# Shashank8834/multimodal-fl-security

Measured on AMD Instinct MI355X. Metric: FL rounds/sec + aggregate-ms, K=128 clients 10M-param multimodal, 1/2/4/8 GPU, higher is better.
Workload: dtype f32 (bf16x6-split MFMA conv/GEMM = fp32 operands; Krum Gram bf16x4 hi/lo split, fp32 accumulate); 1 GPU; C3: Multi-Krum K=128, 20% sign-flip, ResNet-18 img + 1-layer GRU text late fusion, 5 local SGD steps/round; Krum distances reference-exact; preset=C3, model=resnet18-img+gru1-text late-fusion, clients=128, params=11800394, local_steps=5, batch=32, defense=krum(f=25, multi_k=64), attack=sign_flip, attackers=25, client_chunk=128, exchange=alltoall, krum_distances=reference-exact (fp32 torch.norm accumulation, D bit-identical to krum.py:89-97), training_phase=one captured HIP graph per round; local updates = one flr_train_clients_ex call

## Files before the change

### multimodal-fl-security_amd/csrc/agg_pairwise_ref.hip

```cpp
#include <cstdint>
#include <type_traits>
#include <utility>
#include <vector>

#include "flr_common.h"

namespace flr {
namespace pwref {

typedef float f32x4 __attribute__((ext_vector_type(4)));
typedef int i32x16 __attribute__((ext_vector_type(16)));

constexpr int IW = 4;
constexpr int JW = 16;
constexpr int SB = 32;
constexpr int OFF_W = (SB / IW) * (SB / JW);
constexpr int DIAG_W = SB / IW;
constexpr int CS = 64;
constexpr int NQ = CS / 4;
constexpr int RPD = 256 / CS;
constexpr int SROWS = 20;
#ifndef FLR_REF_NSTAGE
#define FLR_REF_NSTAGE 8
#endif
constexpr int NSTAGE = FLR_REF_NSTAGE;
constexpr int STAGE = SROWS * CS;
constexpr int64_t XC_CAP = int64_t(8) << 30;
constexpr int64_t XC_SLACK = 4096;
constexpr int64_t XC_GROUP = (int64_t)NSTAGE * CS;
static_assert(CS == 64 && NQ == 16, "x_i layout: 16 lanes x 4 steps per chunk");
static_assert(NSTAGE % 2 == 0 && NSTAGE >= 4, "two register buffers");
static_assert((NSTAGE - 1) * CS * 4 <= XC_SLACK, "the prefetch past a stream stays inside the slack");
static_assert((NSTAGE - 1) * STAGE * 4 < 65536, "ds_read_b128's 16-bit offset reaches every stage");
static_assert(NSTAGE * STAGE * 4 > 163840 / 5, "LDS caps the CU at four workgroups: one wave per SIMD");
template <bool DIAG>
struct Staging {
  static constexpr int DPW = (DIAG ? SROWS : JW) / RPD;
  static constexpr int OPB = DPW + 1;
  static_assert((NSTAGE - 2) * OPB + 1 < 64, "vmcnt counts to 63");
};

__host__ __device__ constexpr int slot_swz(int row) { return row & 15; }

__host__ __device__ inline int tiles_before(int Y) { return DIAG_W * Y * Y; }
__host__ __device__ inline int ntiles_of(int K) { return tiles_before((K + SB - 1) / SB); }
struct Tile {
  int X, Y, g, h;
  bool diag;
};
__host__ __device__ inline Tile tile_of(int t) {
  int Y = 0;
  while (tiles_before(Y + 1) <= t) ++Y;
  const int local = t - tiles_before(Y);
  Tile r;
  r.Y = Y;
  if (local < Y * OFF_W) {
    r.X = local / OFF_W;
    r.g = (local % OFF_W) >> 1;
    r.h = local & 1;
    r.diag = false;
  } else {
    r.X = Y;
    r.g = local - Y * OFF_W;
    r.h = 0;
    r.diag = true;
  }
  return r;
}
__host__ __device__ inline int tile_of_pair(int i, int j) {
  const int X = i / SB, Y = j / SB;
  if (X < Y) return tiles_before(Y) + X * OFF_W + 2 * ((i % SB) / IW) + (j % SB) / JW;
  const int a = i % SB, b = j % SB, o = b - a;
  const int ii = o <= SB / 2 ? a : b;
  return tiles_before(Y) + Y * OFF_W + ii / IW;
}

constexpr int TW = 256;
constexpr int TROW = TW + 4;
struct WaveRuns {
  static constexpr int MAX = 48;
  int n;
  int64_t w0[MAX], pre[MAX + 1];
};
__global__ __launch_bounds__(256) void chain_transpose_kernel(const float* __restrict__ X, int64_t ldx, int64_t r0,
                                                              int64_t steps, int64_t ldc, float* __restrict__ Xc,
                                                              const WaveRuns runs) {
  __shared__ __attribute__((aligned(16))) float t[4 * 8 * TROW];
  const int k = blockIdx.y, wave = threadIdx.x >> 6, lane = threadIdx.x & 63;
  const int64_t q = (int64_t)blockIdx.x * 4 + wave;
  if (q >= runs.pre[runs.n]) return;
  int r = 0;
  while (q >= runs.pre[r + 1]) ++r;
  const int64_t s0 = (runs.w0[r] + q - runs.pre[r]) * TW;
  const int nv = (int)(steps - s0 < TW ? steps - s0 : TW);
  const float* src = X + (int64_t)k * ldx + 8 * (r0 + s0);
  float* tw = t + wave * 8 * TROW;
  const int h = lane & 1, sl = lane >> 1;
  f32x4 v[8];
  if (nv == TW) {
#pragma unroll
    for (int q = 0; q < 8; ++q) v[q] = __builtin_nontemporal_load(reinterpret_cast<const f32x4*>(src) + 64 * q + lane);
  } else {
#pragma unroll
    for (int q = 0; q < 8; ++q)
      v[q] = 32 * q + sl < nv ? reinterpret_cast<const f32x4*>(src)[64 * q + lane] : f32x4{0.f, 0.f, 0.f, 0.f};
  }
#pragma unroll
  for (int q = 0; q < 8; ++q)
#pragma unroll
    for (int e = 0; e < 4; ++e) tw[(4 * h + e) * TROW + 32 * q + sl] = v[q][e];
  asm volatile("s_waitcnt lgkmcnt(0)" ::: "memory");
  float* dst = Xc + (int64_t)k * 8 * ldc + s0 + 4 * lane;
  if (nv == TW) {
#pragma unroll
    for (int c = 0; c < 8; ++c)
      *reinterpret_cast<f32x4*>(dst + (int64_t)c * ldc) = *reinterpret_cast<const f32x4*>(tw + c * TROW + 4 * lane);
  } else {
    for (int c = 0; c < 8; ++c)
      for (int e = 0; e < 4 && 4 * lane + e < nv; ++e) dst[(int64_t)c * ldc + e] = tw[c * TROW + 4 * lane + e];
  }
}

constexpr int TAP_CO = 32;
constexpr int TAP_ROWS = 288;
static_assert(TAP_CO * TAP_ROWS < (1 << 14), "dense write items exact in fp32");
template <int KKT, bool VEC>
__global__ __launch_bounds__(256) void tap_chain_kernel(const float* __restrict__ X, int64_t ldx, int64_t off,
                                                        int Cout, int Cin, int KKr, int64_t r0, int64_t steps,
                                                        int64_t ldc, float* __restrict__ Xc,
                                                        const float* __restrict__ gdead, uint64_t dead, int nneg) {
  constexpr int TCO = TAP_CO, TROWS = TAP_ROWS;
  __shared__ float tile[TROWS][TCO + 1];
  const int KK = KKT > 0 ? KKT : KKr;
  const int CI = TROWS / KK;
  const int nci_t = (Cin + CI - 1) / CI, ntiles = (int)gridDim.x;
  const int x = (int)(blockIdx.x & 7), j = (int)(blockIdx.x >> 3);
  const int tl = x * (ntiles / 8) + min(x, ntiles % 8) + j;
  const int co0 = (tl / nci_t) * TCO, ci0 = (tl % nci_t) * CI;
  const int nci = min(CI, Cin - ci0), nco_v = min(TCO, Cout - co0);
  const int k = blockIdx.y;
  const float* row = X + (int64_t)k * ldx + off;
  const float* grow = gdead ? gdead + off : row;
  const float gs = k < nneg ? -1.f : 1.f;
  auto is_dead = [&](int t) { return t < 64 && ((dead >> t) & 1); };
  auto src = [&](int t) { return is_dead(t) ? grow : row; };
  auto sgn = [&](int t) { return is_dead(t) ? gs : 1.f; };
  const int nrows = KK * CI;
  if constexpr (VEC) {
    constexpr int LPR = TCO / 4, RPP = 256 / LPR;
    const int sub = threadIdx.x % LPR, rr = threadIdx.x / LPR;
    constexpr int IT = (TROWS + RPP - 1) / RPP;
    f32x4 v[IT];
#pragma unroll
    for (int q = 0; q < IT; ++q) {
      const int r = rr + RPP * q, t = r / CI, ci = r - t * CI;
      const int64_t e = ((int64_t)t * Cin + ci0 + ci) * Cout + co0 + 4 * sub;
      if (!(r < nrows && ci < nci))
        v[q] = f32x4{0.f, 0.f, 0.f, 0.f};
      else if (is_dead(t))
        v[q] = *reinterpret_cast<const f32x4*>(grow + e) * gs;
      else
        v[q] = __builtin_nontemporal_load(reinterpret_cast<const f32x4*>(row + e));
    }
#pragma unroll
    for (int q = 0; q < IT; ++q) {
      const int r = rr + RPP * q;
      if (r < nrows)
#pragma unroll
        for (int e = 0; e < 4; ++e) tile[r][4 * sub + e] = v[q][e];
    }
  } else {
    for (int e = threadIdx.x; e < nrows * TCO; e += 256) {
      const int co = e % TCO, r = e / TCO, t = r / CI, ci = r % CI;
      if (ci < nci && co < nco_v) tile[r][co] = src(t)[((int64_t)t * Cin + ci0 + ci) * Cout + co0 + co] * sgn(t);
    }
  }
  __syncthreads();
  const int64_t L = (int64_t)nci * KK;
  const int64_t ulo = 8 * r0, uhi = 8 * (r0 + steps);
  float* out = Xc + (int64_t)k * 8 * ldc;
  {
    const int64_t CL = (int64_t)Cin * KK;
    const int64_t ufirst = off + ((int64_t)co0 * Cin + ci0) * KK;
    if (CL % 8 == 0 && L % 8 == 0 && ufirst >= ulo && ufirst + (nco_v - 1) * CL + L <= uhi) {
      const int Li = (int)L, m = Li / 8, a0 = (int)(ufirst & 7);
      const int64_t sb0 = (ufirst >> 3) - r0, CLs = CL / 8;
      const float inv_L = 1.f / (float)Li, inv_m = 1.f / (float)m;
      const int n = nco_v * Li;
#pragma unroll 4
      for (int i = threadIdx.x; i < n; i += 256) {
        const int co = (int)(((float)i + 0.5f) * inv_L);
        const int q = i - co * Li;
        const int c = (int)(((float)q + 0.5f) * inv_m);
        const int jj = q - c * m;
        const int dc = (c - a0) & 7;
        const int rel = dc + 8 * jj, ci = rel / KK, t = rel - ci * KK;
        out[(int64_t)c * ldc + sb0 + co * CLs + ((a0 + dc) >> 3) + jj] = tile[t * CI + ci][co];
      }
      return;
    }
  }
  static_assert(TROWS / 8 + 1 <= 64, "a run's steps fit its slots");
#pragma unroll 4
  for (int i = threadIdx.x; i < nco_v * 512; i += 256) {
    const int ns = i & 63, c = (i >> 6) & 7, co = i >> 9;
    const int64_t u0 = off + ((int64_t)(co0 + co) * Cin + ci0) * KK;
    const int64_t u = 8 * ((u0 >> 3) + ns) + c;
    if (u >= u0 && u < u0 + L && u >= ulo && u < uhi) {
      const int rel = (int)(u - u0), ci = rel / KK, t = rel - ci * KK;
      out[(int64_t)c * ldc + ((u >> 3) - r0)] = tile[t * CI + ci][co];
    }
  }
}

#ifndef FLR_REF_ABL
#define FLR_REF_ABL 0
#endif
#if FLR_REF_ABL == 1
#define FLR_CHAIN16(A, B, C, D, NOP) \
  NOP \
  "v_sub_f32 %[t0], %[x0], %[j0]\n\t" \
  "v_sub_f32 %[t1], %[x1], %[j1]\n\t" \
  "v_fmac_f32 %[acc], %[t0], %[t0]\n\t" \
  "v_sub_f32 %[t2], %[x2], %[j2]\n\t" \
  "v_fmac_f32 %[acc], %[t1], %[t1]\n\t" \
  "v_sub_f32 %[t0], %[x3], %[j3]\n\t" \
  "v_fmac_f32 %[acc], %[t2], %[t2]\n\t" \
  "v_sub_f32 %[t1], %[x0], %[j4]\n\t" \
  "v_fmac_f32 %[acc], %[t0], %[t0]\n\t" \
  "v_sub_f32 %[t2], %[x1], %[j5]\n\t" \
  "v_fmac_f32 %[acc], %[t1], %[t1]\n\t" \
  "v_sub_f32 %[t0], %[x2], %[j6]\n\t" \
  "v_fmac_f32 %[acc], %[t2], %[t2]\n\t" \
  "v_sub_f32 %[t1], %[x3], %[j7]\n\t" \
  "v_fmac_f32 %[acc], %[t0], %[t0]\n\t" \
  "v_sub_f32 %[t2], %[x0], %[j8]\n\t" \
  "v_fmac_f32 %[acc], %[t1], %[t1]\n\t" \
  "v_sub_f32 %[t0], %[x1], %[j9]\n\t" \
  "v_fmac_f32 %[acc], %[t2], %[t2]\n\t" \
  "v_sub_f32 %[t1], %[x2], %[j10]\n\t" \
  "v_fmac_f32 %[acc], %[t0], %[t0]\n\t" \
  "v_sub_f32 %[t2], %[x3], %[j11]\n\t" \
  "v_fmac_f32 %[acc], %[t1], %[t1]\n\t" \
  "v_sub_f32 %[t0], %[x0], %[j12]\n\t" \
  "v_fmac_f32 %[acc], %[t2], %[t2]\n\t" \
  "v_sub_f32 %[t1], %[x1], %[j13]\n\t" \
  "v_fmac_f32 %[acc], %[t0], %[t0]\n\t" \
  "v_sub_f32 %[t2], %[x2], %[j14]\n\t" \
  "v_fmac_f32 %[acc], %[t1], %[t1]\n\t" \
  "v_sub_f32 %[t0], %[x3], %[j15]\n\t" \
  "v_fmac_f32 %[acc], %[t2], %[t2]\n\t" \
  "v_fmac_f32 %[acc], %[t0], %[t0]\n\t"
#else
#define FLR_CHAIN16(A, B, C, D, NOP) \
  NOP \
  "v_sub_f32_dpp %[t0], %[x0], %[j0] row_newbcast:" #A " row_mask:0xf bank_mask:0xf\n\t" \
  "v_sub_f32_dpp %[t1], %[x1], %[j1] row_newbcast:" #A " row_mask:0xf bank_mask:0xf\n\t" \
  "v_fmac_f32 %[acc], %[t0], %[t0]\n\t" \
  "v_sub_f32_dpp %[t2], %[x2], %[j2] row_newbcast:" #A " row_mask:0xf bank_mask:0xf\n\t" \
  "v_fmac_f32 %[acc], %[t1], %[t1]\n\t" \
  "v_sub_f32_dpp %[t0], %[x3], %[j3] row_newbcast:" #A " row_mask:0xf bank_mask:0xf\n\t" \
  "v_fmac_f32 %[acc], %[t2], %[t2]\n\t" \
  "v_sub_f32_dpp %[t1], %[x0], %[j4] row_newbcast:" #B " row_mask:0xf bank_mask:0xf\n\t" \
  "v_fmac_f32 %[acc], %[t0], %[t0]\n\t" \
  "v_sub_f32_dpp %[t2], %[x1], %[j5] row_newbcast:" #B " row_mask:0xf bank_mask:0xf\n\t" \
  "v_fmac_f32 %[acc], %[t1], %[t1]\n\t" \
  "v_sub_f32_dpp %[t0], %[x2], %[j6] row_newbcast:" #B " row_mask:0xf bank_mask:0xf\n\t" \
  "v_fmac_f32 %[acc], %[t2], %[t2]\n\t" \
  "v_sub_f32_dpp %[t1], %[x3], %[j7] row_newbcast:" #B " row_mask:0xf bank_mask:0xf\n\t" \
  "v_fmac_f32 %[acc], %[t0], %[t0]\n\t" \
  "v_sub_f32_dpp %[t2], %[x0], %[j8] row_newbcast:" #C " row_mask:0xf bank_mask:0xf\n\t" \
  "v_fmac_f32 %[acc], %[t1], %[t1]\n\t" \
  "v_sub_f32_dpp %[t0], %[x1], %[j9] row_newbcast:" #C " row_mask:0xf bank_mask:0xf\n\t" \
  "v_fmac_f32 %[acc], %[t2], %[t2]\n\t" \
  "v_sub_f32_dpp %[t1], %[x2], %[j10] row_newbcast:" #C " row_mask:0xf bank_mask:0xf\n\t" \
  "v_fmac_f32 %[acc], %[t0], %[t0]\n\t" \
  "v_sub_f32_dpp %[t2], %[x3], %[j11] row_newbcast:" #C " row_mask:0xf bank_mask:0xf\n\t" \
  "v_fmac_f32 %[acc], %[t1], %[t1]\n\t" \
  "v_sub_f32_dpp %[t0], %[x0], %[j12] row_newbcast:" #D " row_mask:0xf bank_mask:0xf\n\t" \
  "v_fmac_f32 %[acc], %[t2], %[t2]\n\t" \
  "v_sub_f32_dpp %[t1], %[x1], %[j13] row_newbcast:" #D " row_mask:0xf bank_mask:0xf\n\t" \
  "v_fmac_f32 %[acc], %[t0], %[t0]\n\t" \
  "v_sub_f32_dpp %[t2], %[x2], %[j14] row_newbcast:" #D " row_mask:0xf bank_mask:0xf\n\t" \
  "v_fmac_f32 %[acc], %[t1], %[t1]\n\t" \
  "v_sub_f32_dpp %[t0], %[x3], %[j15] row_newbcast:" #D " row_mask:0xf bank_mask:0xf\n\t" \
  "v_fmac_f32 %[acc], %[t2], %[t2]\n\t" \
  "v_fmac_f32 %[acc], %[t0], %[t0]\n\t"
#endif
#define FLR_CHAIN_BLOCK(b, A, B, C, D, NOP)                                                                 \
  asm volatile(FLR_CHAIN16(A, B, C, D, NOP)                                                                \
               : [acc] "+v"(acc), [t0] "=&v"(t0), [t1] "=&v"(t1), [t2] "=&v"(t2)                        \
               : [x0] "v"(xv[0]), [x1] "v"(xv[1]), [x2] "v"(xv[2]), [x3] "v"(xv[3]), [j0] "v"(v[4 * (b) + 0][0]), [j1] "v"(v[4 * (b) + 0][1]), [j2] "v"(v[4 * (b) + 0][2]), [j3] "v"(v[4 * (b) + 0][3]), [j4] "v"(v[4 * (b) + 1][0]), [j5] "v"(v[4 * (b) + 1][1]), [j6] "v"(v[4 * (b) + 1][2]), [j7] "v"(v[4 * (b) + 1][3]), [j8] "v"(v[4 * (b) + 2][0]), [j9] "v"(v[4 * (b) + 2][1]), [j10] "v"(v[4 * (b) + 2][2]), [j11] "v"(v[4 * (b) + 2][3]), [j12] "v"(v[4 * (b) + 3][0]), [j13] "v"(v[4 * (b) + 3][1]), [j14] "v"(v[4 * (b) + 3][2]), [j15] "v"(v[4 * (b) + 3][3]))
__device__ __forceinline__ float chain_chunk(f32x4 xv, const f32x4 (&v)[NQ], float acc) {
  static_assert(NQ == 16, "four blocks of 16 steps");
  float t0, t1, t2;
  FLR_CHAIN_BLOCK(0, 0, 1, 2, 3, "s_nop 1\n\t");
  FLR_CHAIN_BLOCK(1, 4, 5, 6, 7, "");
  FLR_CHAIN_BLOCK(2, 8, 9, 10, 11, "");
  FLR_CHAIN_BLOCK(3, 12, 13, 14, 15, "");
  return acc;
}
#undef FLR_CHAIN_BLOCK
#undef FLR_CHAIN16

#define FLR_STEP2(XA, XB, J, L, TA, TB, PA, PB) \
  "v_sub_f32_dpp %[" #TA "], %[" #XA "], %[" #J "] row_newbcast:" #L " row_mask:0xf bank_mask:0xf\n\t" \
  "v_sub_f32_dpp %[" #TB "], %[" #XB "], %[" #J "] row_newbcast:" #L " row_mask:0xf bank_mask:0xf\n\t" \
  "v_fmac_f32 %[acc], %[" #PA "], %[" #PA "]\n\t" \
  "v_fmac_f32 %[acc2], %[" #PB "], %[" #PB "]\n\t"
#define FLR_STEP2_FIRST(XA, XB, J, L, TA, TB) \
  "v_sub_f32_dpp %[" #TA "], %[" #XA "], %[" #J "] row_newbcast:" #L " row_mask:0xf bank_mask:0xf\n\t" \
  "v_sub_f32_dpp %[" #TB "], %[" #XB "], %[" #J "] row_newbcast:" #L " row_mask:0xf bank_mask:0xf\n\t"
#define FLR_CHAIN16_2(A, B, C, D, NOP) \
  NOP \
  FLR_STEP2_FIRST(x0, y0, j0, A, a0, b0) \
  FLR_STEP2(x1, y1, j1, A, a1, b1, a0, b0) FLR_STEP2(x2, y2, j2, A, a0, b0, a1, b1) \
  FLR_STEP2(x3, y3, j3, A, a1, b1, a0, b0) FLR_STEP2(x0, y0, j4, B, a0, b0, a1, b1) \
  FLR_STEP2(x1, y1, j5, B, a1, b1, a0, b0) FLR_STEP2(x2, y2, j6, B, a0, b0, a1, b1) \
  FLR_STEP2(x3, y3, j7, B, a1, b1, a0, b0) FLR_STEP2(x0, y0, j8, C, a0, b0, a1, b1) \
  FLR_STEP2(x1, y1, j9, C, a1, b1, a0, b0) FLR_STEP2(x2, y2, j10, C, a0, b0, a1, b1) \
  FLR_STEP2(x3, y3, j11, C, a1, b1, a0, b0) FLR_STEP2(x0, y0, j12, D, a0, b0, a1, b1) \
  FLR_STEP2(x1, y1, j13, D, a1, b1, a0, b0) FLR_STEP2(x2, y2, j14, D, a0, b0, a1, b1) \
  FLR_STEP2(x3, y3, j15, D, a1, b1, a0, b0) \
  "v_fmac_f32 %[acc], %[a1], %[a1]\n\t" \
  "v_fmac_f32 %[acc2], %[b1], %[b1]\n\t"
#define FLR_CHAIN_BLOCK2(b, A, B, C, D, NOP)                                                                   \
  asm volatile(FLR_CHAIN16_2(A, B, C, D, NOP)                                                                 \
               : [acc] "+v"(acc), [acc2] "+v"(acc2), [a0] "=&v"(a0), [b0] "=&v"(b0), [a1] "=&v"(a1),          \
                 [b1] "=&v"(b1)                                                                              \
               : [x0] "v"(xv[0]), [x1] "v"(xv[1]), [x2] "v"(xv[2]), [x3] "v"(xv[3]), [y0] "v"(yv[0]),           \
                 [y1] "v"(yv[1]), [y2] "v"(yv[2]), [y3] "v"(yv[3]), [j0] "v"(v[4 * (b) + 0][0]),              \
                 [j1] "v"(v[4 * (b) + 0][1]), [j2] "v"(v[4 * (b) + 0][2]), [j3] "v"(v[4 * (b) + 0][3]),        \
                 [j4] "v"(v[4 * (b) + 1][0]), [j5] "v"(v[4 * (b) + 1][1]), [j6] "v"(v[4 * (b) + 1][2]),        \
                 [j7] "v"(v[4 * (b) + 1][3]), [j8] "v"(v[4 * (b) + 2][0]), [j9] "v"(v[4 * (b) + 2][1]),        \
                 [j10] "v"(v[4 * (b) + 2][2]), [j11] "v"(v[4 * (b) + 2][3]), [j12] "v"(v[4 * (b) + 3][0]),     \
                 [j13] "v"(v[4 * (b) + 3][1]), [j14] "v"(v[4 * (b) + 3][2]), [j15] "v"(v[4 * (b) + 3][3]))
__device__ __forceinline__ void chain_chunk2(f32x4 xv, f32x4 yv, const f32x4 (&v)[NQ], float& acc, float& acc2) {
  float a0, b0, a1, b1;
  FLR_CHAIN_BLOCK2(0, 0, 1, 2, 3, "s_nop 1\n\t");
  FLR_CHAIN_BLOCK2(1, 4, 5, 6, 7, "");
  FLR_CHAIN_BLOCK2(2, 8, 9, 10, 11, "");
  FLR_CHAIN_BLOCK2(3, 12, 13, 14, 15, "");
}
#undef FLR_CHAIN_BLOCK2
#undef FLR_CHAIN16_2
#undef FLR_STEP2_FIRST
#undef FLR_STEP2

template <class F, int... U>
__device__ __forceinline__ void static_for(F&& f, std::integer_sequence<int, U...>) {
  (f(std::integral_constant<int, U>{}), ...);
}

template <bool DIAG, int NST = NSTAGE, bool TWO = false>
__device__ __forceinline__ void ref_chain_tile(float* lds, const Tile T, const int c, const float* __restrict__ Xc,
                                               int64_t ldc, int K, int64_t steps, int first,
                                               float* __restrict__ A) {
  using S = Staging<DIAG>;
  static_assert(!(TWO && DIAG), "two chains per lane on off-diagonal tiles only");
  static_assert(NST % 2 == 0 && NST >= 4, "two register buffers");
  constexpr int NXI = TWO ? 2 : 1;
  constexpr int OPB = S::DPW + NXI;
  static_assert((NST - 2) * OPB + NXI < 64, "vmcnt counts to 63");
  const int lane = threadIdx.x & 63, r = lane >> 4, jl = lane & 15;
  int i, j, srow;
  bool keep = true;
  if (DIAG) {
    const int a = IW * T.g + r, o = jl + 1;
    i = SB * T.X + a;
    j = SB * T.X + ((a + o) & (SB - 1));
    srow = r + jl;
    keep = o < SB / 2 || a < SB / 2;
  } else {
    i = SB * T.X + (TWO ? 2 * IW : IW) * T.g + r;
    j = SB * T.Y + JW * T.h + jl;
    srow = jl;
  }
  const int i2 = i + IW;
  const bool valid2 = TWO && i2 < K && j < K;
  const bool valid = keep && i < K && j < K;
  const int lo = i < j ? i : j, hi = i < j ? j : i;
  const int64_t rs = 8 * ldc;

  float acc = 0.f, acc2 = 0.f;
  if (!first) {
    const float* ap = A + ((int64_t)c * K + (lo < K ? lo : K - 1)) * K + (hi < K ? hi : K - 1);
    asm volatile("global_load_dword %0, %1, off\n\ts_waitcnt vmcnt(0)" : "=v"(acc) : "v"(ap) : "memory");
    acc = valid ? acc : 0.f;
    if constexpr (TWO) {
      const float* ap2 = A + ((int64_t)c * K + (i2 < K ? i2 : K - 1)) * K + (j < K ? j : K - 1);
      asm volatile("global_load_dword %0, %1, off\n\ts_waitcnt vmcnt(0)" : "=v"(acc2) : "v"(ap2) : "memory");
      acc2 = valid2 ? acc2 : 0.f;
    }
  }

  const int jrow0 = DIAG ? SB * T.X : min(SB * T.Y + JW * T.h, K - 1);
  const char* sbj = reinterpret_cast<const char*>(Xc + (int64_t)jrow0 * rs + (int64_t)c * ldc) - 2048;
  uint32_t voj[S::DPW];
#pragma unroll
  for (int u = 0; u < S::DPW; ++u) {
    const int s = RPD * u + lane / NQ;
    int gj = DIAG ? SB * T.X + ((IW * T.g + 1 + s) & (SB - 1)) : SB * T.Y + JW * T.h + s;
    gj = gj < K ? gj : K - 1;
    voj[u] = (uint32_t)((int64_t)(gj - jrow0) * rs * 4 + 16 * ((lane % NQ) ^ slot_swz(s)) - 1024 * (u - 2) + 2048);
  }
  const int irow0 = min(DIAG ? SB * T.X + IW * T.g : i - r, K - 1);
  const char* sbi = reinterpret_cast<const char*>(Xc + (int64_t)irow0 * rs + (int64_t)c * ldc);
  const uint32_t voi = (uint32_t)((int64_t)((i < K ? i : K - 1) - irow0) * rs * 4 + 16 * jl);
  const uint32_t voi2 = (uint32_t)((int64_t)((i2 < K ? i2 : K - 1) - irow0) * rs * 4 + 16 * jl);
  static_assert(XC_GROUP % (NST * CS) == 0, "trips inside the zero fill");
  const int ngroup = (int)((steps + NST * CS - 1) / (NST * CS));
  auto issue = [&](int ch, int slot, f32x4& x, f32x4& x2) {
    const int64_t co = (int64_t)ch * CS * 4;
    if (FLR_REF_ABL == 3) return;
    const char* sb = sbj + co;
    const uint32_t m = (uint32_t)(uintptr_t)lds + 4 * slot * STAGE + 2048;
#define FLR_DMA(n, off) "global_load_lds_dwordx4 %[v" #n "], %[sb] offset:" #off "\n\t"
    if constexpr (S::DPW == 5)
      asm volatile("s_mov_b32 m0, %[m]\n\ts_nop 0\n\t" FLR_DMA(0, -2048) FLR_DMA(1, -1024) FLR_DMA(2, 0)
                       FLR_DMA(3, 1024) FLR_DMA(4, 2048)
                   :
                   : [m] "s"(m), [sb] "s"(sb), [v0] "v"(voj[0]), [v1] "v"(voj[1]), [v2] "v"(voj[2]), [v3] "v"(voj[3]),
                     [v4] "v"(voj[S::DPW - 1])
                   : "memory");
    else
      asm volatile("s_mov_b32 m0, %[m]\n\ts_nop 0\n\t" FLR_DMA(0, -2048) FLR_DMA(1, -1024) FLR_DMA(2, 0)
                       FLR_DMA(3, 1024)
                   :
                   : [m] "s"(m), [sb] "s"(sb), [v0] "v"(voj[0]), [v1] "v"(voj[1]), [v2] "v"(voj[2]), [v3] "v"(voj[3])
                   : "memory");
#undef FLR_DMA
    static_assert(S::DPW == 4 || S::DPW == 5, "the DMA statements above");
    asm volatile("global_load_dwordx4 %0, %1, %2" : "=v"(x) : "v"(voi), "s"(sbi + co) : "memory");
    if constexpr (TWO) asm volatile("global_load_dwordx4 %0, %1, %2" : "=v"(x2) : "v"(voi2), "s"(sbi + co) : "memory");
  };
  const int rsw = slot_swz(srow);
  uint32_t ra[NQ];
#pragma unroll
  for (int q = 0; q < NQ; ++q) ra[q] = (uint32_t)(uintptr_t)(lds + srow * CS + 4 * (q ^ rsw));
  auto rows = [](auto st, f32x4(&v)[NQ], const uint32_t(&a)[NQ]) {
#pragma unroll
    for (int q = 0; q < NQ; ++q)
      if (FLR_REF_ABL != 2)
        asm volatile("ds_read_b128 %0, %1 offset:%2" : "=v"(v[q]) : "v"(a[q]), "n"(decltype(st)::value * STAGE * 4)
                     : "memory");
  };

  f32x4 va[NQ], vb[NQ];
  f32x4 xs[NST], xs2[NST];
  auto body = [&](auto U, int ch, f32x4(&vc)[NQ], f32x4(&vn)[NQ]) {
    constexpr int u = decltype(U)::value;
    asm volatile("s_waitcnt vmcnt(%0)" ::"n"((NST - 3) * OPB + NXI) : "memory");
    asm volatile("s_waitcnt lgkmcnt(0)" ::: "memory");
    asm volatile("" : "+v"(vc[0]), "+v"(vc[1]), "+v"(vc[2]), "+v"(vc[3]), "+v"(vc[4]), "+v"(vc[5]), "+v"(vc[6]),
                 "+v"(vc[7]), "+v"(vc[8]), "+v"(vc[9]), "+v"(vc[10]), "+v"(vc[11]), "+v"(vc[12]), "+v"(vc[13]),
                 "+v"(vc[14]), "+v"(vc[15]), "+v"(xs[u]));
    if constexpr (TWO) asm volatile("" : "+v"(xs2[u]));
    issue(ch + NST - 1, (u + NST - 1) % NST, xs[(u + NST - 1) % NST], xs2[(u + NST - 1) % NST]);
    rows(std::integral_constant<int, (u + 1) % NST>{}, vn, ra);
    if constexpr (TWO)
      chain_chunk2(xs[u], xs2[u], vc, acc, acc2);
    else if (FLR_REF_ABL != 5)
      acc = chain_chunk(xs[u], vc, acc);
  };
#pragma unroll
  for (int u = 0; u < NST - 1; ++u) issue(u, u, xs[u], xs2[u]);
  asm volatile("s_waitcnt vmcnt(%0)" ::"n"((NST - 2) * OPB + NXI) : "memory");
  rows(std::integral_constant<int, 0>{}, va, ra);
  for (int ch = 0; ch < ngroup * NST; ch += NST)
    static_for(
        [&](auto U) {
          constexpr int u = decltype(U)::value;
          if constexpr (u % 2 == 0)
            body(U, ch + u, va, vb);
          else
            body(U, ch + u, vb, va);
        },
        std::make_integer_sequence<int, NST>{});
  asm volatile("s_waitcnt vmcnt(0) lgkmcnt(0)" ::: "memory");
  if (valid) A[((int64_t)c * K + lo) * K + hi] = acc;
  if (valid2) A[((int64_t)c * K + i2) * K + j] = acc2;
}

__global__ __launch_bounds__(64) void ref_chain_kernel(const float* __restrict__ Xc, int64_t ldc, int K,
                                                       int64_t steps, int t0, int first, float* __restrict__ A) {
  __shared__ __attribute__((aligned(16))) float lds[NSTAGE * STAGE];
  const int c = (int)(blockIdx.x & 7);
  const Tile T = tile_of(t0 + (int)(blockIdx.x >> 3));
  if (T.diag)
    ref_chain_tile<true>(lds, T, c, Xc, ldc, K, steps, first, A);
  else
    ref_chain_tile<false>(lds, T, c, Xc, ldc, K, steps, first, A);
}

constexpr int NST2 = 4;
__host__ __device__ inline int tiles2_before(int Y) { return 4 * Y * (Y + 1); }
__host__ __device__ inline int ntiles2_of(int K) { return tiles2_before((K + SB - 1) / SB); }
__host__ __device__ inline Tile tile2_of(int t) {
  int Y = 0;
  while (tiles2_before(Y + 1) <= t) ++Y;
  const int local = t - tiles2_before(Y);
  Tile r;
  r.Y = Y;
  if (local < 8 * Y) {
    r.X = local / 8;
    r.g = (local % 8) >> 1;
    r.h = local & 1;
    r.diag = false;
  } else {
    r.X = Y;
    r.g = local - 8 * Y;
    r.h = 0;
    r.diag = true;
  }
  return r;
}
__global__ __launch_bounds__(64, 2) void ref_chain2_kernel(const float* __restrict__ Xc, int64_t ldc, int K,
                                                           int64_t steps, int first, float* __restrict__ A) {
  __shared__ __attribute__((aligned(16))) float lds[NST2 * STAGE];
  const int c = (int)(blockIdx.x & 7);
  const Tile T = tile2_of((int)(blockIdx.x >> 3));
  if (T.diag)
    ref_chain_tile<true, NST2, false>(lds, T, c, Xc, ldc, K, steps, first, A);
  else
    ref_chain_tile<false, NST2, true>(lds, T, c, Xc, ldc, K, steps, first, A);
}

inline bool use_two_chains(int64_t K) {
  const char* e = flr::knob("FLR_REF_2I");
  return e && e[0] == '1' && K > SB;
}

constexpr int QJ = 64;
constexpr int QTB = 16;
constexpr int QD = 8;
static_assert(XC_GROUP % (4 * QTB) == 0 && XC_GROUP % (4 * QD) == 0, "padded segments hold whole tiles / trips");
__host__ __device__ inline int64_t quad_rows(int64_t K) { return (K + QJ - 1) / QJ * QJ; }
__host__ __device__ inline int quad_ni(int q, int K, int ni) {
  const int a = QJ / ni * (q + 1), b = (K + ni - 1) / ni;
  return a < b ? a : b;
}
inline int64_t quad_slack(int64_t K) { return (QD + 4) * quad_rows(K) * 16; }
inline int quad_ntiles(int K, int ni) {
  int n = 0;
  for (int q = 0; q * QJ < K; ++q) n += quad_ni(q, K, ni);
  return n;
}

__global__ __launch_bounds__(256) void quad_transpose_kernel(const float* __restrict__ X, int64_t ldx, int K,
                                                             int64_t r0, int64_t steps, int64_t NB, int64_t Kp,
                                                             float* __restrict__ Xq) {
  __shared__ f32x4 t[QTB][QTB * 8 + 1];
  const int tid = threadIdx.x;
  const int64_t b0 = (int64_t)blockIdx.x * QTB;
  const int k0 = blockIdx.y * QTB;
  const int64_t u0 = 8 * (r0 + 4 * b0), uend = 8 * (r0 + steps);
  f32x4 v[8];
#pragma unroll
  for (int q = 0; q < 8; ++q) {
    const int idx = q * 256 + tid, row = idx >> 7, p = idx & 127;
    const int64_t u = u0 + 4 * p;
    v[q] = (k0 + row < K && u < uend)
               ? __builtin_nontemporal_load(reinterpret_cast<const f32x4*>(X + (int64_t)(k0 + row) * ldx + u))
               : f32x4{0.f, 0.f, 0.f, 0.f};
  }
#pragma unroll
  for (int q = 0; q < 8; ++q) {
    const int idx = q * 256 + tid;
    t[idx >> 7][idx & 127] = v[q];
  }
  __syncthreads();
  const int k = tid & 15, bl = tid >> 4;
  if (k0 + k >= K) return;
  f32x4 w[8];
#pragma unroll
  for (int q = 0; q < 8; ++q) w[q] = t[k][8 * bl + q];
  float* out = Xq + ((b0 + bl) * Kp + k0 + k) * 4;
#pragma unroll
  for (int c = 0; c < 8; ++c) {
    const int h = c >> 2, m = c & 3;
    *reinterpret_cast<f32x4*>(out + (int64_t)c * NB * Kp * 4) = f32x4{w[h][m], w[2 + h][m], w[4 + h][m], w[6 + h][m]};
  }
}

template <int E>
__device__ __forceinline__ void sgpr_step(float (&acc)[4], const i32x16& g0, const i32x16&, float xjv) {
  float t0, t1;
  asm volatile(
      "v_sub_f32 %[t0], %[s0], %[x]\n\t"
      "v_sub_f32 %[t1], %[s1], %[x]\n\t"
      "v_fmac_f32 %[a0], %[t0], %[t0]\n\t"
      "v_sub_f32 %[t0], %[s2], %[x]\n\t"
      "v_fmac_f32 %[a1], %[t1], %[t1]\n\t"
      "v_sub_f32 %[t1], %[s3], %[x]\n\t"
      "v_fmac_f32 %[a2], %[t0], %[t0]\n\t"
      "v_fmac_f32 %[a3], %[t1], %[t1]\n\t"
      : [a0] "+v"(acc[0]), [a1] "+v"(acc[1]), [a2] "+v"(acc[2]), [a3] "+v"(acc[3]), [t0] "=&v"(t0), [t1] "=&v"(t1)
      : [s0] "s"(g0[E]), [s1] "s"(g0[4 + E]), [s2] "s"(g0[8 + E]), [s3] "s"(g0[12 + E]), [x] "v"(xjv));
}
template <int E>
__device__ __forceinline__ void sgpr_step(float (&acc)[8], const i32x16& g0, const i32x16& g1, float xjv) {
  float t0, t1;
  asm volatile(
      "v_sub_f32 %[t0], %[s0], %[x]\n\t"
      "v_sub_f32 %[t1], %[s1], %[x]\n\t"
      "v_fmac_f32 %[a0], %[t0], %[t0]\n\t"
      "v_sub_f32 %[t0], %[s2], %[x]\n\t"
      "v_fmac_f32 %[a1], %[t1], %[t1]\n\t"
      "v_sub_f32 %[t1], %[s3], %[x]\n\t"
      "v_fmac_f32 %[a2], %[t0], %[t0]\n\t"
      "v_sub_f32 %[t0], %[s4], %[x]\n\t"
      "v_fmac_f32 %[a3], %[t1], %[t1]\n\t"
      "v_sub_f32 %[t1], %[s5], %[x]\n\t"
      "v_fmac_f32 %[a4], %[t0], %[t0]\n\t"
      "v_sub_f32 %[t0], %[s6], %[x]\n\t"
      "v_fmac_f32 %[a5], %[t1], %[t1]\n\t"
      "v_sub_f32 %[t1], %[s7], %[x]\n\t"
      "v_fmac_f32 %[a6], %[t0], %[t0]\n\t"
      "v_fmac_f32 %[a7], %[t1], %[t1]\n\t"
      : [a0] "+v"(acc[0]), [a1] "+v"(acc[1]), [a2] "+v"(acc[2]), [a3] "+v"(acc[3]), [a4] "+v"(acc[4]),
        [a5] "+v"(acc[5]), [a6] "+v"(acc[6]), [a7] "+v"(acc[7]), [t0] "=&v"(t0), [t1] "=&v"(t1)
      : [s0] "s"(g0[E]), [s1] "s"(g0[4 + E]), [s2] "s"(g0[8 + E]), [s3] "s"(g0[12 + E]), [s4] "s"(g1[E]),
        [s5] "s"(g1[4 + E]), [s6] "s"(g1[8 + E]), [s7] "s"(g1[12 + E]), [x] "v"(xjv));
}

#ifndef FLR_REF_S_ABL
#define FLR_REF_S_ABL 0
#endif
template <int NI, int BT>
__global__ __launch_bounds__(64) void ref_chain_s_kernel(const float* __restrict__ Xq, int64_t NB, int64_t Kp, int K,
                                                         int first, float* __restrict__ A) {
  static_assert(NI == 4 || NI == 8, "the step forms above");
  constexpr int NL = NI * BT / 4;
  static_assert(QD % (2 * BT) == 0, "whole ping-pong pairs of buffers per trip");
  const int c = (int)(blockIdx.x & 7), lane = threadIdx.x;
  int t = (int)(blockIdx.x >> 3), q = 0;
  for (int n = quad_ni(0, K, NI); t >= n; n = quad_ni(q, K, NI)) {
    t -= n;
    ++q;
  }
  const int i0 = NI * t, j = QJ * q + lane;
  const float* __restrict__ base = Xq + (int64_t)c * NB * Kp * 4;
  float acc[NI];
  if (first) {
#pragma unroll
    for (int r = 0; r < NI; ++r) acc[r] = 0.f;
  } else {
#pragma unroll
    for (int r = 0; r < NI; ++r) {
      const float* ap = A + ((int64_t)c * K + i0 + r) * K + (j < K ? j : K - 1);
      asm volatile("global_load_dword %0, %1, off" : "=v"(acc[r]) : "v"(ap) : "memory");
    }
    if constexpr (NI == 4)
      asm volatile("s_waitcnt vmcnt(0)" : "+v"(acc[0]), "+v"(acc[1]), "+v"(acc[2]), "+v"(acc[3]) : : "memory");
    else
      asm volatile("s_waitcnt vmcnt(0)"
                   : "+v"(acc[0]), "+v"(acc[1]), "+v"(acc[2]), "+v"(acc[3]), "+v"(acc[4]), "+v"(acc[5]),
                     "+v"(acc[6]), "+v"(acc[7])
                   :
                   : "memory");
#pragma unroll
    for (int r = 0; r < NI; ++r) acc[r] = (i0 + r < j && j < K) ? acc[r] : 0.f;
  }
  const int64_t bb = Kp * 16;
  const uint32_t voff = (uint32_t)j * 16;
  const char* pjn = reinterpret_cast<const char*>(base);
  const char* pin = reinterpret_cast<const char*>(base) + (int64_t)i0 * 16;
  auto ldj = [&](f32x4& x) {
    asm volatile("global_load_dwordx4 %0, %1, %2" : "=v"(x) : "v"(voff), "s"(pjn) : "memory");
    pjn += bb;
    asm volatile("" : "+s"(pjn));
  };
  auto ldi = [&](i32x16(&buf)[NL]) {
    const char* pu = pin;
#pragma unroll
    for (int u = 0; u < BT; ++u) {
#pragma unroll
      for (int h = 0; h < NI / 4; ++h)
        asm volatile("s_load_dwordx16 %0, %1, %2" : "=s"(buf[u * (NI / 4) + h]) : "s"(pu), "n"(64 * h) : "memory");
      pu += bb;
      asm volatile("" : "+s"(pu));
    }
    pin = pu;
  };
  f32x4 xj[QD];
  i32x16 xa[NL], xb[NL];
#pragma unroll
  for (int u = 0; u < QD; ++u) ldj(xj[u]);
  ldi(xa);
  auto trip = [&](auto U0, const i32x16(&cur)[NL], i32x16(&nxt)[NL]) {
    constexpr int u0 = decltype(U0)::value;
    if (FLR_REF_S_ABL != 2 && FLR_REF_S_ABL != 4) asm volatile("s_waitcnt lgkmcnt(0)" ::: "memory");
    if (FLR_REF_S_ABL != 2) ldi(nxt);
#pragma unroll
    for (int v = 0; v < BT; ++v) {
      f32x4& x = xj[u0 + v];
      if (FLR_REF_S_ABL != 1) asm volatile("s_waitcnt vmcnt(%0)" ::"n"(QD - 1) : "memory");
      asm volatile("" : "+v"(x));
      const i32x16& g0 = cur[v * (NI / 4)];
      const i32x16& g1 = cur[v * (NI / 4) + (NI / 4) - 1];
      if (FLR_REF_S_ABL != 3) {
        sgpr_step<0>(acc, g0, g1, x[0]);
        sgpr_step<1>(acc, g0, g1, x[1]);
        sgpr_step<2>(acc, g0, g1, x[2]);
        sgpr_step<3>(acc, g0, g1, x[3]);
      }
      if (FLR_REF_S_ABL != 1) ldj(x);
    }
  };
  for (int64_t b0 = 0; b0 < NB; b0 += QD)
    static_for(
        [&](auto P) {
          constexpr int p = decltype(P)::value;
          trip(std::integral_constant<int, 2 * BT * p>{}, xa, xb);
          trip(std::integral_constant<int, 2 * BT * p + BT>{}, xb, xa);
        },
        std::make_integer_sequence<int, QD / (2 * BT)>{});
  asm volatile("s_waitcnt vmcnt(0) lgkmcnt(0)" ::: "memory");
#pragma unroll
  for (int r = 0; r < NI; ++r) {
    const int i = i0 + r;
    if (i < j && j < K) A[((int64_t)c * K + i) * K + j] = acc[r];
  }
}

constexpr int WCB = 8;
constexpr int WNS = 4;
static_assert(WCB % 8 == 0 && (XC_GROUP / 4) % WCB == 0, "two DMAs per wave per chunk; whole chunks per segment");
__host__ __device__ inline int wg_groups(int q, int K) { return (quad_ni(q, K, 8) + 3) / 4; }
inline int wg_ntiles(int K) {
  int n = 0;
  for (int q = 0; q * QJ < K; ++q) n += wg_groups(q, K);
  return n;
}
template <int E>
__device__ __forceinline__ void vgpr_step(float (&acc)[8], const f32x4 (&xi)[8], float xjv) {
  float t0, t1;
  asm volatile(
      "v_sub_f32 %[t0], %[s0], %[x]\n\t"
      "v_sub_f32 %[t1], %[s1], %[x]\n\t"
      "v_fmac_f32 %[a0], %[t0], %[t0]\n\t"
      "v_sub_f32 %[t0], %[s2], %[x]\n\t"
      "v_fmac_f32 %[a1], %[t1], %[t1]\n\t"
      "v_sub_f32 %[t1], %[s3], %[x]\n\t"
      "v_fmac_f32 %[a2], %[t0], %[t0]\n\t"
      "v_sub_f32 %[t0], %[s4], %[x]\n\t"
      "v_fmac_f32 %[a3], %[t1], %[t1]\n\t"
      "v_sub_f32 %[t1], %[s5], %[x]\n\t"
      "v_fmac_f32 %[a4], %[t0], %[t0]\n\t"
      "v_sub_f32 %[t0], %[s6], %[x]\n\t"
      "v_fmac_f32 %[a5], %[t1], %[t1]\n\t"
      "v_sub_f32 %[t1], %[s7], %[x]\n\t"
      "v_fmac_f32 %[a6], %[t0], %[t0]\n\t"
      "v_fmac_f32 %[a7], %[t1], %[t1]\n\t"
      : [a0] "+v"(acc[0]), [a1] "+v"(acc[1]), [a2] "+v"(acc[2]), [a3] "+v"(acc[3]), [a4] "+v"(acc[4]),
        [a5] "+v"(acc[5]), [a6] "+v"(acc[6]), [a7] "+v"(acc[7]), [t0] "=&v"(t0), [t1] "=&v"(t1)
      : [s0] "v"(xi[0][E]), [s1] "v"(xi[1][E]), [s2] "v"(xi[2][E]), [s3] "v"(xi[3][E]), [s4] "v"(xi[4][E]),
        [s5] "v"(xi[5][E]), [s6] "v"(xi[6][E]), [s7] "v"(xi[7][E]), [x] "v"(xjv));
}

template <bool XL>
__global__ __launch_bounds__(256, 3) void ref_chain_w_kernel(const float* __restrict__ Xq, int64_t NB, int64_t Kp,
                                                             int K, int first, float* __restrict__ A) {
  constexpr int SJ = WCB * QJ * 16;
  constexpr int SI = XL ? WCB * 32 * 16 : 0;
  constexpr int NDMA = XL ? 3 : 2;
  __shared__ __attribute__((aligned(16))) float xs[WNS * (SJ + SI) / 4];
  const int c = (int)(blockIdx.x & 7), lane = threadIdx.x & 63;
  const int wave = __builtin_amdgcn_readfirstlane((int)(threadIdx.x >> 6));
  int t = (int)(blockIdx.x >> 3), q = 0;
  for (int n = wg_groups(0, K); t >= n; n = wg_groups(q, K)) {
    t -= n;
    ++q;
  }
  const int a = 4 * t + wave, na = quad_ni(q, K, 8);
  const bool live = a < na;
  const int i0 = 8 * (live ? a : na - 1), j = QJ * q + lane;
  const float* __restrict__ base = Xq + (int64_t)c * NB * Kp * 4;
  float acc[8];
  if (first || !live) {
#pragma unroll
    for (int r = 0; r < 8; ++r) acc[r] = 0.f;
  } else {
#pragma unroll
    for (int r = 0; r < 8; ++r) {
      const float* ap = A + ((int64_t)c * K + i0 + r) * K + (j < K ? j : K - 1);
      asm volatile("global_load_dword %0, %1, off" : "=v"(acc[r]) : "v"(ap) : "memory");
    }
    asm volatile("s_waitcnt vmcnt(0)"
                 : "+v"(acc[0]), "+v"(acc[1]), "+v"(acc[2]), "+v"(acc[3]), "+v"(acc[4]), "+v"(acc[5]), "+v"(acc[6]),
                   "+v"(acc[7])
                 :
                 : "memory");
#pragma unroll
    for (int r = 0; r < 8; ++r) acc[r] = (i0 + r < j && j < K) ? acc[r] : 0.f;
  }
  const int64_t bb = Kp * 16;
  const int64_t nch = NB / WCB;
  const char* jsrc = reinterpret_cast<const char*>(base) + (int64_t)(QJ * q) * 16;
  const char* isrc = reinterpret_cast<const char*>(base) + (int64_t)(32 * t) * 16;
  const uint32_t vj = (uint32_t)lane * 16;
  const uint32_t vi = (uint32_t)(((lane >> 5) * Kp + (lane & 31)) * 16);
  const uint32_t lds0 = (uint32_t)(uintptr_t)xs;
  auto dma = [&](int64_t ch) {
    const int64_t cc = ch < nch ? ch : nch - 1;
    const uint32_t sb = lds0 + (uint32_t)((int)(ch % WNS) * (SJ + SI));
#pragma unroll
    for (int v = 0; v < 2; ++v) {
      const int blk = 2 * wave + v;
      const char* src = jsrc + (cc * WCB + blk) * bb;
      const uint32_t m = sb + (uint32_t)(blk * QJ * 16);
      asm volatile("s_mov_b32 m0, %[m]\n\ts_nop 0\n\tglobal_load_lds_dwordx4 %[v], %[s] offset:0"
                   :
                   : [m] "s"(m), [v] "v"(vj), [s] "s"(src)
                   : "memory");
    }
    if constexpr (XL) {
      const char* src = isrc + (cc * WCB + 2 * wave) * bb;
      const uint32_t m = sb + SJ + (uint32_t)(2 * wave * 32 * 16);
      asm volatile("s_mov_b32 m0, %[m]\n\ts_nop 0\n\tglobal_load_lds_dwordx4 %[v], %[s] offset:0"
                   :
                   : [m] "s"(m), [v] "v"(vi), [s] "s"(src)
                   : "memory");
    }
  };
  const char* pin = reinterpret_cast<const char*>(base) + (int64_t)i0 * 16;
  auto ldi = [&](i32x16& lo, i32x16& hi) {
    asm volatile("s_load_dwordx16 %0, %2, 0x0\n\ts_load_dwordx16 %1, %2, 0x40" : "=s"(lo), "=s"(hi) : "s"(pin) : "memory");
    pin += bb;
    asm volatile("" : "+s"(pin));
  };
  auto rdj = [&](f32x4& x, uint32_t addr, auto U) {
    asm volatile("ds_read_b128 %0, %1 offset:%2" : "=v"(x) : "v"(addr), "n"(decltype(U)::value * QJ * 16) : "memory");
  };
  auto rdi = [&](f32x4(&x)[8], uint32_t addr, auto U) {
#pragma unroll
    for (int r = 0; r < 8; ++r)
      asm volatile("ds_read_b128 %0, %1 offset:%2"
                   : "=v"(x[r])
                   : "v"(addr), "n"(SJ + decltype(U)::value * 32 * 16 + 16 * r)
                   : "memory");
  };
  i32x16 al, ah, bl, bh;
  f32x4 j0, j1, ia[8], ib[8];
#pragma unroll
  for (int p = 0; p < WNS - 1; ++p) dma(p);
  if constexpr (!XL) ldi(al, ah);
  auto body = [&](auto U, uint32_t sbase, uint32_t ibase, f32x4& xc, f32x4& xn, const i32x16& cl,
                  const i32x16& ch_, i32x16& nl, i32x16& nh, f32x4(&ic)[8], f32x4(&in)[8]) {
    constexpr int u = decltype(U)::value;
    if constexpr (XL) {
      asm volatile("s_waitcnt lgkmcnt(0)"
                   : "+v"(xc), "+v"(ic[0]), "+v"(ic[1]), "+v"(ic[2]), "+v"(ic[3]), "+v"(ic[4]), "+v"(ic[5]),
                     "+v"(ic[6]), "+v"(ic[7])
                   :
                   : "memory");
      if constexpr (u + 1 < WCB) {
        rdj(xn, sbase, std::integral_constant<int, u + 1>{});
        rdi(in, ibase, std::integral_constant<int, u + 1>{});
      }
      vgpr_step<0>(acc, ic, xc[0]);
      vgpr_step<1>(acc, ic, xc[1]);
      vgpr_step<2>(acc, ic, xc[2]);
      vgpr_step<3>(acc, ic, xc[3]);
    } else {
      asm volatile("s_waitcnt lgkmcnt(0)" : "+v"(xc) : : "memory");
      ldi(nl, nh);
      if constexpr (u + 1 < WCB) rdj(xn, sbase, std::integral_constant<int, u + 1>{});
      sgpr_step<0>(acc, cl, ch_, xc[0]);
      sgpr_step<1>(acc, cl, ch_, xc[1]);
      sgpr_step<2>(acc, cl, ch_, xc[2]);
      sgpr_step<3>(acc, cl, ch_, xc[3]);
    }
  };
  static_assert(WCB % 2 == 0, "x_i / x_j ping-pong");
  for (int64_t ch = 0; ch < nch; ++ch) {
    asm volatile("s_waitcnt vmcnt(%0)\n\ts_barrier" ::"n"(NDMA * (WNS - 2)) : "memory");
    dma(ch + WNS - 1);
    const uint32_t st = lds0 + (uint32_t)((int)(ch % WNS) * (SJ + SI));
    const uint32_t sbase = st + vj;
    const uint32_t ibase = st + (uint32_t)(wave * 8 * 16);
    rdj(j0, sbase, std::integral_constant<int, 0>{});
    if constexpr (XL) rdi(ia, ibase, std::integral_constant<int, 0>{});
    static_for(
        [&](auto P) {
          constexpr int p = decltype(P)::value;
          body(std::integral_constant<int, 2 * p>{}, sbase, ibase, j0, j1, al, ah, bl, bh, ia, ib);
          body(std::integral_constant<int, 2 * p + 1>{}, sbase, ibase, j1, j0, bl, bh, al, ah, ib, ia);
        },
        std::make_integer_sequence<int, WCB / 2>{});
  }
  asm volatile("s_waitcnt vmcnt(0) lgkmcnt(0)" ::: "memory");
  if (live) {
#pragma unroll
    for (int r = 0; r < 8; ++r) {
      const int i = i0 + r;
      if (i < j && j < K) A[((int64_t)c * K + i) * K + j] = acc[r];
    }
  }
}

inline bool use_quad(int64_t K, int64_t ntaps, bool all_tiles) {
  if (!all_tiles || ntaps > 0 || K <= QJ) return false;
  const char* e = flr::knob("FLR_REF_SGPR");
  if (e && e[0] == '0') return false;
  if (e && e[0] == '1') return true;
  return K >= 480;
}

struct TailCols {
  int64_t c[8];
};
__global__ void ref_finish_kernel(const float* __restrict__ A, int chains, const float* __restrict__ X,
                                  const TailCols tc, int K, int64_t P, int64_t ldx, int64_t R, int t0, int t1,
                                  double* __restrict__ D) {
  const int64_t idx = (int64_t)blockIdx.x * blockDim.x + threadIdx.x;
  if (idx >= (int64_t)K * K) return;
  const int i = (int)(idx / K), j = (int)(idx % K);
  if (i == j) {
    D[idx] = 0.0;
    return;
  }
  if (i > j) return;
  const int tile = tile_of_pair(i, j);
  double v = 0.0;
  if (tile >= t0 && tile < t1) {
    float s = 0.f;
    if (chains) {
      const int64_t kk = (int64_t)K * K, p = (int64_t)i * K + j;
      s = A[p];
#pragma unroll
      for (int c = 1; c < 8; ++c) s = add_rn(s, A[c * kk + p]);
    }
    const float* xi = X + (int64_t)i * ldx;
    const float* xj = X + (int64_t)j * ldx;
    int64_t t = R * 8;
    auto col = [&](int64_t c) { return tc.c[c - R * 8]; };
    if (t + 4 <= P)
      for (const int64_t e = t + 4; t < e; ++t) {
        const float d = xi[col(t)] - xj[col(t)];
        s = add_rn(s, mul_rn(d, d));
      }
    for (; t < P; ++t) {
      const float d = xi[col(t)] - xj[col(t)];
      s = __builtin_fmaf(d, d, s);
    }
    v = (double)sqrt_rn(s);
  }
  D[(int64_t)i * K + j] = v;
  D[(int64_t)j * K + i] = v;
}

inline size_t a_bytes(int64_t K) { return align_up((size_t)(8 * K * K) * 4, 256); }

}
}

using namespace flr;
using namespace flr::pwref;

extern "C" size_t flr_pairwise_l2_reference_workspace(int64_t K, int64_t P) {
  if (K < 1 || P < 0) return 0;
  const int64_t R = P / 8;
  size_t n = a_bytes(K);
  if (K < 2 || R == 0) return n;
  const int64_t Rc = (R + XC_GROUP - 1) / XC_GROUP * XC_GROUP;
  const int64_t per_step = (K > QJ ? quad_rows(K) : K) * 8 * 4;
  const int64_t nseg = (per_step * Rc + XC_CAP - 1) / XC_CAP;
  const int64_t Rs = ((R + nseg - 1) / nseg + XC_GROUP - 1) / XC_GROUP * XC_GROUP;
  return n + (size_t)(per_step * Rs + XC_SLACK + (K > QJ ? quad_slack(K) : 0));
}

extern "C" int flr_pairwise_l2_reference_tiles(int64_t K) {
  if (K < 2 || K > (1 << 15)) return 0;
  return ntiles_of((int)K);
}

static WaveRuns wave_runs(const int64_t* taps, int64_t ntaps, int64_t r0, int64_t steps) {
  const int64_t nw = (steps + TW - 1) / TW;
  std::vector<std::pair<int64_t, int64_t>> v;
  int64_t b = 0;
  for (int64_t w = 0; w < nw; ++w) {
    const int64_t u0 = 8 * (r0 + w * TW), u1 = u0 + 8 * TW;
    while (b < ntaps && taps[4 * b] + taps[4 * b + 1] * taps[4 * b + 2] * taps[4 * b + 3] <= u0) ++b;
    const bool inside = b < ntaps && u0 >= taps[4 * b] &&
                        u1 <= taps[4 * b] + taps[4 * b + 1] * taps[4 * b + 2] * taps[4 * b + 3];
    if (inside) continue;
    if (!v.empty() && v.back().second == w)
      v.back().second = w + 1;
    else
      v.push_back({w, w + 1});
  }
  while ((int)v.size() > WaveRuns::MAX) {
    size_t best = 1;
    for (size_t i = 2; i < v.size(); ++i)
      if (v[i].first - v[i - 1].second < v[best].first - v[best - 1].second) best = i;
    v[best - 1].second = v[best].second;
    v.erase(v.begin() + (int64_t)best);
  }
  WaveRuns wr;
  wr.n = (int)v.size();
  wr.pre[0] = 0;
  for (int i = 0; i < wr.n; ++i) {
    wr.w0[i] = v[i].first;
    wr.pre[i + 1] = wr.pre[i] + (v[i].second - v[i].first);
  }
  return wr;
}

static int run_chains(const float* X, int64_t K, int64_t steps_total, int64_t ldx, const int64_t* taps, int64_t ntaps,
                      const uint64_t* dead, const float* gdead, int64_t nneg, int first, float* A, void* ws,
                      size_t ws_bytes, int t0, int t1, hipStream_t st) {
  const size_t na = a_bytes(K);
  if (ws_bytes < na) return FLR_ERR_WORKSPACE;
  const int64_t R = steps_total;
  if (ws_bytes < na + (size_t)XC_SLACK) return FLR_ERR_WORKSPACE;
  if (use_quad(K, ntaps, t0 == 0 && t1 == ntiles_of((int)K))) {
    const int64_t Kp = quad_rows(K), qstep = Kp * 8 * 4;
    const char* rows_knob = flr::knob("FLR_REF_SGPR_ROWS");
    const bool eight = rows_knob && rows_knob[0] == '8';
    const char* form_knob = flr::knob("FLR_REF_SGPR_FORM");
    const bool wg = !(form_knob && form_knob[0] == 'w' && form_knob[1] == 'a');
    const bool xl = !(form_knob && form_knob[0] == 's');
    if (ws_bytes < na + (size_t)(XC_SLACK + quad_slack(K))) return FLR_ERR_WORKSPACE;
    const int64_t cap =
        (int64_t)((ws_bytes - na - XC_SLACK - quad_slack(K)) / (size_t)qstep) / XC_GROUP * XC_GROUP;
    if (cap < XC_GROUP) return FLR_ERR_WORKSPACE;
    const int64_t nseg = (R + cap - 1) / cap;
    const int64_t Rs = ((R + nseg - 1) / nseg + XC_GROUP - 1) / XC_GROUP * XC_GROUP;
    float* Xq = reinterpret_cast<float*>(reinterpret_cast<char*>(ws) + na);
    for (int64_t seg = 0; seg < nseg; ++seg) {
      const int64_t r0 = seg * Rs, steps = (R - r0 < Rs) ? R - r0 : Rs;
      if (steps <= 0) break;
      const int64_t NB = (steps + XC_GROUP - 1) / XC_GROUP * XC_GROUP / 4;
      hipLaunchKernelGGL(quad_transpose_kernel, dim3((unsigned)(NB / QTB), (unsigned)((K + QTB - 1) / QTB)), dim3(256),
                         0, st, X, ldx, (int)K, r0, steps, NB, Kp, Xq);
      int rc = launch_status("quad_transpose_kernel");
      if (rc != FLR_OK) return rc;
      const int fst = (first && seg == 0) ? 1 : 0;
      if (wg && xl)
        hipLaunchKernelGGL(ref_chain_w_kernel<true>, dim3((unsigned)(8 * wg_ntiles((int)K))), dim3(256), 0, st, Xq, NB,
                           Kp, (int)K, fst, A);
      else if (wg)
        hipLaunchKernelGGL(ref_chain_w_kernel<false>, dim3((unsigned)(8 * wg_ntiles((int)K))), dim3(256), 0, st, Xq,
                           NB, Kp, (int)K, fst, A);
      else if (eight)
        hipLaunchKernelGGL((ref_chain_s_kernel<8, 1>), dim3((unsigned)(8 * quad_ntiles((int)K, 8))), dim3(64), 0, st,
                           Xq, NB, Kp, (int)K, fst, A);
      else
        hipLaunchKernelGGL((ref_chain_s_kernel<4, 2>), dim3((unsigned)(8 * quad_ntiles((int)K, 4))), dim3(64), 0, st,
                           Xq, NB, Kp, (int)K, fst, A);
      if ((rc = launch_status("ref_chain_s_kernel")) != FLR_OK) return rc;
    }
    return FLR_OK;
  }
  const int64_t per_step = K * 8 * 4;
  const int64_t ldc = (int64_t)((ws_bytes - na - XC_SLACK) / (size_t)per_step) / XC_GROUP * XC_GROUP;
  if (ldc < XC_GROUP) return FLR_ERR_WORKSPACE;
  const int64_t nseg = (R + ldc - 1) / ldc;
  const int64_t Rs = ((R + nseg - 1) / nseg + XC_GROUP - 1) / XC_GROUP * XC_GROUP;
  float* Xc = reinterpret_cast<float*>(reinterpret_cast<char*>(ws) + na);
  for (int64_t seg = 0; seg < nseg; ++seg) {
    const int64_t r0 = seg * Rs, steps = (R - r0 < Rs) ? R - r0 : Rs;
    if (steps <= 0) break;
    const WaveRuns runs = wave_runs(taps, ntaps, r0, steps);
    int rc = FLR_OK;
    if (runs.pre[runs.n] > 0) {
      hipLaunchKernelGGL(chain_transpose_kernel, dim3((unsigned)((runs.pre[runs.n] + 3) / 4), (unsigned)K), dim3(256),
                         0, st, X, ldx, r0, steps, ldc, Xc, runs);
      if ((rc = launch_status("chain_transpose_kernel")) != FLR_OK) return rc;
    }
    for (int64_t b = 0; b < ntaps; ++b) {
      const int64_t off = taps[4 * b], co = taps[4 * b + 1], ci = taps[4 * b + 2], kk = taps[4 * b + 3];
      if (off + co * ci * kk <= 8 * r0 || off >= 8 * (r0 + steps)) continue;
      const int64_t tiles = (co + TAP_CO - 1) / TAP_CO * ((ci + TAP_ROWS / kk - 1) / (TAP_ROWS / kk));
      const bool vec = off % 4 == 0 && co % TAP_CO == 0;
      auto kern = kk == 9 ? (vec ? tap_chain_kernel<9, true> : tap_chain_kernel<9, false>)
                : kk == 1 ? (vec ? tap_chain_kernel<1, true> : tap_chain_kernel<1, false>)
                          : (vec ? tap_chain_kernel<0, true> : tap_chain_kernel<0, false>);
      const uint64_t dm = dead ? dead[b] : 0;
      hipLaunchKernelGGL(kern, dim3((unsigned)tiles, (unsigned)K), dim3(256), 0, st, X, ldx, off, (int)co, (int)ci,
                         (int)kk, r0, steps, ldc, Xc, dm ? gdead : nullptr, dm, (int)std::min<int64_t>(nneg, K));
      if ((rc = launch_status("tap_chain_kernel")) != FLR_OK) return rc;
    }
    const int64_t padded = (steps + XC_GROUP - 1) / XC_GROUP * XC_GROUP;
    if (padded > steps &&
        hipMemset2DAsync(Xc + steps, (size_t)ldc * 4, 0, (size_t)(padded - steps) * 4, (size_t)(K * 8), st) != hipSuccess)
      return FLR_ERR_HIP;
    if (t0 == 0 && t1 == ntiles_of((int)K) && use_two_chains(K)) {
      hipLaunchKernelGGL(ref_chain2_kernel, dim3(8 * ntiles2_of((int)K)), dim3(64), 0, st, Xc, ldc, (int)K, steps,
                         (first && seg == 0) ? 1 : 0, A);
      rc = launch_status("ref_chain2_kernel");
    } else {
      hipLaunchKernelGGL(ref_chain_kernel, dim3(8 * (t1 - t0)), dim3(64), 0, st, Xc, ldc, (int)K, steps, t0,
                         (first && seg == 0) ? 1 : 0, A);
      rc = launch_status("ref_chain_kernel");
    }
    if (rc != FLR_OK) return rc;
  }
  return FLR_OK;
}

static int check_rows(const float* X, int64_t K, int64_t n, int64_t ldx) {
  if (K > 1 && n >= 8 && (((reinterpret_cast<uintptr_t>(X) & 15) != 0) || (ldx % 4) != 0)) return FLR_ERR_ARG;
  return FLR_OK;
}

extern "C" int flr_pairwise_l2_reference_tap_dead(const float* X, int64_t K, int64_t P, int64_t ldx,
                                                  const int64_t* taps, int64_t ntaps, const uint64_t* dead,
                                                  const float* gdead, int64_t nneg, double* D, void* ws,
                                                  size_t ws_bytes, int64_t part, int64_t nparts, void* stream) {
  if (K < 1 || P < 0 || ldx < P || !D || (K > 1 && P > 0 && !X) || nparts < 1 || part < 0 || part >= nparts)
    return FLR_ERR_ARG;
  if (K > (1 << 15)) return FLR_ERR_UNSUPPORTED;
  if (ntaps < 0 || (ntaps > 0 && !taps) || nneg < 0) return FLR_ERR_ARG;
  bool any_dead = false;
  for (int64_t b = 0; dead && b < ntaps; ++b) {
    if (taps[4 * b + 3] < 64 && (dead[b] >> taps[4 * b + 3]) != 0) return FLR_ERR_ARG;
    any_dead |= dead[b] != 0;
  }
  if (any_dead && !gdead) return FLR_ERR_ARG;
  for (int64_t b = 0, end = 0; b < ntaps; ++b) {
    const int64_t off = taps[4 * b], co = taps[4 * b + 1], ci = taps[4 * b + 2], kk = taps[4 * b + 3];
    if (off < end || co < 1 || ci < 1 || kk < 1 || kk > TAP_ROWS || co > INT32_MAX || ci > INT32_MAX ||
        off + co * ci * kk > P)
      return FLR_ERR_ARG;
    end = off + co * ci * kk;
  }
  int rc = check_rows(X, K, P, ldx);
  if (rc != FLR_OK) return rc;
  hipStream_t st = as_stream(stream);
  const int64_t R = P / 8;
  if (K > 1 && R > 0 && (!ws || (reinterpret_cast<uintptr_t>(ws) & 255) != 0)) return FLR_ERR_WORKSPACE;
  const int ntiles = K > 1 ? ntiles_of((int)K) : 0;
  const int t0 = (int)(part * ntiles / nparts), t1 = (int)((part + 1) * ntiles / nparts);
  float* A = reinterpret_cast<float*>(ws);
  if (K > 1 && R > 0 && t1 > t0 &&
      (rc = run_chains(X, K, R, ldx, taps, ntaps, any_dead ? dead : nullptr, gdead, nneg, 1, A, ws, ws_bytes, t0, t1,
                       st)) != FLR_OK)
    return rc;
  TailCols tc;
  for (int64_t u = 8 * R; u < 8 * R + 8; ++u) {
    int64_t c = u;
    for (int64_t b = 0; b < ntaps && u < P; ++b) {
      const int64_t off = taps[4 * b], co = taps[4 * b + 1], ci = taps[4 * b + 2], kk = taps[4 * b + 3];
      if (u < off || u >= off + co * ci * kk) continue;
      const int64_t rel = u - off, o = rel / (ci * kk), i = (rel / kk) % ci, t = rel % kk;
      c = off + (t * ci + i) * co + o;
    }
    tc.c[u - 8 * R] = c;
  }
  for (int64_t u = 8 * R; any_dead && u < P; ++u)
    for (int64_t b = 0; b < ntaps; ++b) {
      const int64_t off = taps[4 * b], co = taps[4 * b + 1], ci = taps[4 * b + 2], kk = taps[4 * b + 3];
      if (u < off || u >= off + co * ci * kk) continue;
      const int64_t t = (u - off) % kk;
      if (t < 64 && ((dead[b] >> t) & 1)) return FLR_ERR_ARG;
    }
  const int64_t kk = K * K;
  hipLaunchKernelGGL(ref_finish_kernel, dim3((unsigned)((kk + 255) / 256)), dim3(256), 0, st, A, R > 0 ? 1 : 0, X, tc,
                     (int)K, P, ldx, R, t0, t1, D);
  return launch_status("ref_finish_kernel");
}

extern "C" int flr_pairwise_l2_reference_tap(const float* X, int64_t K, int64_t P, int64_t ldx,
                                             const int64_t* taps, int64_t ntaps, double* D, void* ws, size_t ws_bytes,
                                             int64_t part, int64_t nparts, void* stream) {
  return flr_pairwise_l2_reference_tap_dead(X, K, P, ldx, taps, ntaps, nullptr, nullptr, 0, D, ws, ws_bytes, part,
                                            nparts, stream);
}

extern "C" int flr_pairwise_l2_reference(const float* X, int64_t K, int64_t P, int64_t ldx, double* D, void* ws,
                                         size_t ws_bytes, int64_t part, int64_t nparts, void* stream) {
  return flr_pairwise_l2_reference_tap(X, K, P, ldx, nullptr, 0, D, ws, ws_bytes, part, nparts, stream);
}

extern "C" int flr_pairwise_l2_reference_partial_tap(const float* X, int64_t K, int64_t steps, int64_t ldx,
                                                     const int64_t* taps, int64_t ntaps, int first, void* ws,
                                                     size_t ws_bytes, void* stream) {
  if (K < 1 || steps < 0 || ldx < 8 * steps || (K > 1 && steps > 0 && !X)) return FLR_ERR_ARG;
  if (ntaps < 0 || (ntaps > 0 && !taps)) return FLR_ERR_ARG;
  for (int64_t b = 0, end = 0; b < ntaps; ++b) {
    const int64_t off = taps[4 * b], co = taps[4 * b + 1], ci = taps[4 * b + 2], kk = taps[4 * b + 3];
    if (off < end || co < 1 || ci < 1 || kk < 1 || kk > TAP_ROWS || co > INT32_MAX || ci > INT32_MAX ||
        off + co * ci * kk > 8 * steps)
      return FLR_ERR_ARG;
    end = off + co * ci * kk;
  }
  if (K > (1 << 15)) return FLR_ERR_UNSUPPORTED;
  int rc = check_rows(X, K, 8 * steps, ldx);
  if (rc != FLR_OK) return rc;
  if (!ws || (reinterpret_cast<uintptr_t>(ws) & 255) != 0 || ws_bytes < a_bytes(K)) return FLR_ERR_WORKSPACE;
  hipStream_t st = as_stream(stream);
  float* A = reinterpret_cast<float*>(ws);
  if (K < 2) return FLR_OK;
  if (steps == 0) {
    if (first && hipMemsetAsync(A, 0, (size_t)8 * K * K * 4, st) != hipSuccess)
      return launch_status("reference distances: zero the chains");
    return FLR_OK;
  }
  return run_chains(X, K, steps, ldx, taps, ntaps, nullptr, nullptr, 0, first, A, ws, ws_bytes, 0, ntiles_of((int)K),
                    st);
}

extern "C" int flr_pairwise_l2_reference_partial(const float* X, int64_t K, int64_t steps, int64_t ldx, int first,
                                                 void* ws, size_t ws_bytes, void* stream) {
  return flr_pairwise_l2_reference_partial_tap(X, K, steps, ldx, nullptr, 0, first, ws, ws_bytes, stream);
}

extern "C" int flr_pairwise_l2_reference_finish(const float* Xtail, int64_t K, int64_t ntail, int64_t ldx,
                                                int chains, const void* ws, double* D, void* stream) {
  if (K < 1 || ntail < 0 || ntail > 7 || ldx < ntail || !D || (K > 1 && ntail > 0 && !Xtail) ||
      (K > 1 && chains && !ws))
    return FLR_ERR_ARG;
  if (K > (1 << 15)) return FLR_ERR_UNSUPPORTED;
  TailCols tc;
  for (int u = 0; u < 8; ++u) tc.c[u] = u;
  const int64_t kk = K * K;
  hipLaunchKernelGGL(ref_finish_kernel, dim3((unsigned)((kk + 255) / 256)), dim3(256), 0, as_stream(stream),
                     reinterpret_cast<const float*>(ws), chains ? 1 : 0, Xtail, tc, (int)K, ntail, ldx, (int64_t)0, 0,
                     K > 1 ? ntiles_of((int)K) : 0, D);
  return launch_status("ref_finish_kernel");
}
```

Measured before the change: 15.64 rounds/s.

## Compact dead-tap columns out of Krum chain and stream shared dead values separately

For conv taps whose per-client values come from a shared global (dead) tensor with a sign flip, the live taps are now packed separately in the transposed chain buffer. The dead taps are written once into a shared stream with the doubled value, rather than copied per client. A new dead-pattern chain kernel reads that stream into LDS by DMA and adds its squared terms only for mixed-sign client pairs, pointing other pairs at a zero block. The aim is to cut per-client transpose traffic and chain FMAs on dead taps while keeping the distance accumulation order exact. The cost is much more complexity: region planning, hand-scheduled asm specialised for two tap masks, and an Inf/NaN flag passed to the finish kernel.

```diff
diff --git a/multimodal-fl-security_amd/csrc/agg_pairwise_ref.hip b/multimodal-fl-security_amd/csrc/agg_pairwise_ref.hip
--- a/multimodal-fl-security_amd/csrc/agg_pairwise_ref.hip
+++ b/multimodal-fl-security_amd/csrc/agg_pairwise_ref.hip
@@ -124,15 +124,29 @@
 constexpr int TAP_CO = 32;
 constexpr int TAP_ROWS = 288;
 static_assert(TAP_CO * TAP_ROWS < (1 << 14), "dense write items exact in fp32");
-template <int KKT, bool VEC>
+
+struct DeadPlan {
+  int on;
+  int nl, nd;
+  uint64_t tap, rank;
+};
+__host__ __device__ inline int dead_nib(uint64_t v, int n) { return (int)((v >> (4 * n)) & 15); }
+__host__ __device__ inline int64_t dead_slot(int64_t rel, int t, int n, uint64_t rank) {
+  const int64_t c = rel & 7, s = rel >> 3;
+  return (s + 8 - c) / 9 * n + dead_nib(rank, t);
+}
+
+template <int KKT, bool VEC, bool CMP = false>
 __global__ __launch_bounds__(256) void tap_chain_kernel(const float* __restrict__ X, int64_t ldx, int64_t off,
                                                         int Cout, int Cin, int KKr, int64_t r0, int64_t steps,
                                                         int64_t ldc, float* __restrict__ Xc,
-                                                        const float* __restrict__ gdead, uint64_t dead, int nneg) {
+                                                        const float* __restrict__ gdead, uint64_t dead, int nneg,
+                                                        const DeadPlan dp) {
   constexpr int TCO = TAP_CO, TROWS = TAP_ROWS;
   __shared__ float tile[TROWS][TCO + 1];
   const int KK = KKT > 0 ? KKT : KKr;
-  const int CI = TROWS / KK;
+  const int NR = CMP ? dp.nl : KK;
+  const int CI = TROWS / NR;
   const int nci_t = (Cin + CI - 1) / CI, ntiles = (int)gridDim.x;
   const int x = (int)(blockIdx.x & 7), j = (int)(blockIdx.x >> 3);
   const int tl = x * (ntiles / 8) + min(x, ntiles % 8) + j;
@@ -145,7 +159,8 @@
   auto is_dead = [&](int t) { return t < 64 && ((dead >> t) & 1); };
   auto src = [&](int t) { return is_dead(t) ? grow : row; };
   auto sgn = [&](int t) { return is_dead(t) ? gs : 1.f; };
-  const int nrows = KK * CI;
+  const int nrows = NR * CI;
+  auto tap_of = [&](int tr) { return CMP ? dead_nib(dp.tap, tr) : tr; };
   if constexpr (VEC) {
     constexpr int LPR = TCO / 4, RPP = 256 / LPR;
     const int sub = threadIdx.x % LPR, rr = threadIdx.x / LPR;
@@ -153,11 +168,11 @@
     f32x4 v[IT];
 #pragma unroll
     for (int q = 0; q < IT; ++q) {
-      const int r = rr + RPP * q, t = r / CI, ci = r - t * CI;
+      const int r = rr + RPP * q, tr = r / CI, ci = r - tr * CI, t = tap_of(tr);
       const int64_t e = ((int64_t)t * Cin + ci0 + ci) * Cout + co0 + 4 * sub;
       if (!(r < nrows && ci < nci))
         v[q] = f32x4{0.f, 0.f, 0.f, 0.f};
-      else if (is_dead(t))
+      else if (!CMP && is_dead(t))
         v[q] = *reinterpret_cast<const f32x4*>(grow + e) * gs;
       else
         v[q] = __builtin_nontemporal_load(reinterpret_cast<const f32x4*>(row + e));
@@ -171,11 +186,24 @@
     }
   } else {
     for (int e = threadIdx.x; e < nrows * TCO; e += 256) {
-      const int co = e % TCO, r = e / TCO, t = r / CI, ci = r % CI;
-      if (ci < nci && co < nco_v) tile[r][co] = src(t)[((int64_t)t * Cin + ci0 + ci) * Cout + co0 + co] * sgn(t);
+      const int co = e % TCO, r = e / TCO, t = tap_of(r / CI), ci = r % CI;
+      if (ci < nci && co < nco_v)
+        tile[r][co] = (CMP ? row : src(t))[((int64_t)t * Cin + ci0 + ci) * Cout + co0 + co] * (CMP ? 1.f : sgn(t));
     }
   }
   __syncthreads();
+  if constexpr (CMP) {
+    const int per = nci * dp.nl, n = nco_v * per, p8 = per / 8;
+    const bool deal = per % 8 == 0;
+    float* outl = Xc + (int64_t)k * 8 * ldc;
+    for (int i = threadIdx.x; i < n; i += 256) {
+      const int co = i / per, l = i - co * per, q = deal ? 8 * (l % p8) + l / p8 : l;
+      const int ci = q / dp.nl, lt = q - ci * dp.nl, t = dead_nib(dp.tap, lt);
+      const int64_t rel = ((int64_t)(co0 + co) * Cin + ci0 + ci) * KK + t;
+      outl[(rel & 7) * ldc + dead_slot(rel, t, dp.nl, dp.rank)] = tile[lt * CI + ci][co];
+    }
+    return;
+  }
   const int64_t L = (int64_t)nci * KK;
   const int64_t ulo = 8 * r0, uhi = 8 * (r0 + steps);
   float* out = Xc + (int64_t)k * 8 * ldc;
@@ -352,15 +380,158 @@
   (f(std::integral_constant<int, U>{}), ...);
 }
 
-template <bool DIAG, int NST = NSTAGE, bool TWO = false>
+__global__ __launch_bounds__(256) void zero_slots_kernel(float* __restrict__ Xc, int64_t ldc, int n0, int64_t z0,
+                                                         int64_t z1) {
+  float* row = Xc + (int64_t)blockIdx.x * ldc;
+  const int n = n0 + (int)(z1 - z0);
+  for (int i = threadIdx.x; i < n; i += 256) row[i < n0 ? i : z0 + (i - n0)] = 0.f;
+}
+
+__global__ __launch_bounds__(256) void dead_stream_kernel(const float* __restrict__ g, int64_t off, int Cout, int Cin,
+                                                          const DeadPlan dp, int64_t ldt, float* __restrict__ T,
+                                                          int* __restrict__ flag) {
+  const int64_t idx = (int64_t)blockIdx.x * blockDim.x + threadIdx.x;
+  if (idx >= (int64_t)Cout * Cin * dp.nd) return;
+  const int64_t q = idx / dp.nd;
+  const int t = dead_nib(dp.tap, (int)(idx - q * dp.nd));
+  const int64_t co = q / Cin, ci = q - co * Cin;
+  const float v = g[off + ((int64_t)t * Cin + ci) * Cout + co];
+  if ((__float_as_uint(v) & 0x7f800000u) == 0x7f800000u) *flag = 1;
+  const int64_t rel = q * 9 + t;
+  T[(rel & 7) * ldt + dead_slot(rel, t, dp.nd, dp.rank)] = v + v;
+}
+
+template <int DM>
+struct DeadPat {
+  static constexpr int ND = __builtin_popcount(DM & 0x1ff), NL = 9 - ND;
+  static_assert(ND > 0 && NL > 0 && CS % NL == 0, "whole periods per chunk");
+  static constexpr int PPC = CS / NL;
+  static constexpr int TCH = PPC * ND;
+  static_assert(TCH % 4 == 0, "16-B reads of the dead stream");
+  static constexpr int NQT = TCH / 4;
+  static constexpr int NT = (TCH * 4 + 1023) / 1024;
+  static constexpr bool dead_at(int w) { return (DM >> (8 - w)) & 1; }
+  static constexpr int dead_before(int w) {
+    int n = 0;
+    for (int x = 0; x < w; ++x) n += dead_at(x) ? 1 : 0;
+    return n;
+  }
+};
+constexpr int NSTD = 4;
+#define FLR_FMA(x) "v_fmac_f32 %[acc], %[" #x "], %[" #x "]\n\t"
+#define FLR_SUB(dd, x, j, L) \
+  "v_sub_f32_dpp %[" #dd "], %[" #x "], %[" #j "] row_newbcast:%[" #L "] row_mask:0xf bank_mask:0xf\n\t"
+template <int DM>
+__device__ __forceinline__ float dead_chunk(f32x4 xv, const f32x4 (&v)[NQ], float acc, uint32_t ta) {
+  using Pt = DeadPat<DM>;
+  static_assert(DM == 0x1EF || DM == 0x04F, "the period statements below");
+  constexpr int ND = Pt::ND, NQT = Pt::NQT;
+  constexpr int RQ = NQT < 20 ? NQT : (DM == 0x1EF ? 14 : 20);
+  f32x4 tq[RQ];
+  float d[3];
+  auto readq = [&tq, &ta](auto Q) {
+    constexpr int q = decltype(Q)::value;
+    (void)tq, (void)ta;
+    asm volatile("ds_read_b128 %0, %1 offset:%2" : "=v"(tq[q % RQ]) : "v"(ta), "n"(16 * q) : "memory");
+  };
+  static_for([&readq](auto Q) { readq(Q); }, std::make_integer_sequence<int, RQ>{});
+  asm volatile("s_nop 1\n\t" FLR_SUB(da, x0, j0, L) FLR_SUB(db, x1, j1, L)
+               : [da] "=&v"(d[0]), [db] "=&v"(d[1])
+               : [x0] "v"(xv[0]), [x1] "v"(xv[1]), [j0] "v"(v[0][0]), [j1] "v"(v[0][1]), [L] "n"(0));
+  constexpr int G = DM == 0x1EF ? 2 : 1;
+  static_assert(Pt::PPC % G == 0, "whole groups per chunk");
+  static_for(
+      [&tq, &d, &acc, &readq, &xv, &v](auto PP) {
+        constexpr int pg = decltype(PP)::value, p = G * pg, n0 = ND * p;
+        (void)tq, (void)d, (void)acc, (void)xv, (void)v;
+        constexpr int done = n0 / 4, last = (done + RQ < NQT ? done + RQ : NQT) - 1, need = (n0 + G * ND - 1) / 4;
+        constexpr int cnt = last - need < 15 ? last - need : 15;
+        static_assert(need <= last, "the group's reads were issued");
+#define FLR_T(n) tq[((n0 + (n)) / 4) % RQ][(n0 + (n)) % 4]
+#define FLR_T8(a, b) [t##a##0] "v"(FLR_T(b + 0)), [t##a##1] "v"(FLR_T(b + 1)), [t##a##2] "v"(FLR_T(b + 2)), \
+                     [t##a##3] "v"(FLR_T(b + 3)), [t##a##4] "v"(FLR_T(b + 4)), [t##a##5] "v"(FLR_T(b + 5)), \
+                     [t##a##6] "v"(FLR_T(b + 6)), [t##a##7] "v"(FLR_T(b + 7))
+        if constexpr (DM == 0x1EF) {
+          constexpr int S = p, N = S + 2 < CS ? S + 2 : 0;
+          if constexpr (S + 2 < CS)
+            asm volatile("s_waitcnt lgkmcnt(%[w])\n\t" FLR_FMA(ta0) FLR_FMA(ta1) FLR_FMA(ta2) FLR_FMA(ta3) FLR_FMA(d0)
+                             FLR_SUB(n0, x0, j0, L0) FLR_FMA(ta4) FLR_FMA(ta5) FLR_FMA(ta6) FLR_FMA(ta7)
+                                 FLR_FMA(tb0) FLR_FMA(tb1) FLR_FMA(tb2) FLR_FMA(tb3) FLR_FMA(d1)
+                                     FLR_SUB(d0, x1, j1, L1) FLR_FMA(tb4) FLR_FMA(tb5) FLR_FMA(tb6) FLR_FMA(tb7)
+                         : [acc] "+v"(acc), [d0] "+v"(d[S % 3]), [d1] "+v"(d[(S + 1) % 3]), [n0] "=&v"(d[(S + 2) % 3])
+                         : [x0] "v"(xv[N % 4]), [j0] "v"(v[N / 4][N % 4]), [L0] "n"(N / 4), [x1] "v"(xv[(N + 1) % 4]),
+                           [j1] "v"(v[(N + 1) / 4][(N + 1) % 4]), [L1] "n"((N + 1) / 4), [w] "n"(cnt), FLR_T8(a, 0),
+                           FLR_T8(b, 8));
+          else
+            asm volatile("s_waitcnt lgkmcnt(%[w])\n\t" FLR_FMA(ta0) FLR_FMA(ta1) FLR_FMA(ta2) FLR_FMA(ta3) FLR_FMA(d0)
+                             FLR_FMA(ta4) FLR_FMA(ta5) FLR_FMA(ta6) FLR_FMA(ta7) FLR_FMA(tb0) FLR_FMA(tb1)
+                                 FLR_FMA(tb2) FLR_FMA(tb3) FLR_FMA(d1) FLR_FMA(tb4) FLR_FMA(tb5) FLR_FMA(tb6)
+                                     FLR_FMA(tb7)
+                         : [acc] "+v"(acc)
+                         : [d0] "v"(d[S % 3]), [d1] "v"(d[(S + 1) % 3]), [w] "n"(cnt), FLR_T8(a, 0), FLR_T8(b, 8));
+        } else {
+          constexpr int S = 4 * p;
+          float &da = d[S % 3], &db = d[(S + 1) % 3], &dc = d[(S + 2) % 3];
+          if constexpr (S + 4 < CS)
+            asm volatile("s_waitcnt lgkmcnt(%[w])\n\t" FLR_FMA(da) FLR_SUB(dc, x2, j2, L0) FLR_FMA(db)
+                             FLR_SUB(da, x3, j3, L0) FLR_FMA(t0) FLR_FMA(dc) FLR_SUB(db, x0, j4, L1) FLR_FMA(da)
+                                 FLR_SUB(dc, x1, j5, L1) FLR_FMA(t1) FLR_FMA(t2) FLR_FMA(t3) FLR_FMA(t4)
+                         : [acc] "+v"(acc), [da] "+v"(da), [db] "+v"(db), [dc] "+v"(dc)
+                         : [x0] "v"(xv[0]), [x1] "v"(xv[1]), [x2] "v"(xv[2]), [x3] "v"(xv[3]), [j2] "v"(v[p][2]),
+                           [j3] "v"(v[p][3]), [j4] "v"(v[p + 1 < NQ ? p + 1 : p][0]),
+                           [j5] "v"(v[p + 1 < NQ ? p + 1 : p][1]), [L0] "n"(p), [L1] "n"(p + 1), [w] "n"(cnt),
+                           [t0] "v"(FLR_T(0)), [t1] "v"(FLR_T(1)), [t2] "v"(FLR_T(2)), [t3] "v"(FLR_T(3)),
+                           [t4] "v"(FLR_T(4)));
+          else
+            asm volatile("s_waitcnt lgkmcnt(%[w])\n\t" FLR_FMA(da) FLR_SUB(dc, x2, j2, L0) FLR_FMA(db)
+                             FLR_SUB(da, x3, j3, L0) FLR_FMA(t0) FLR_FMA(dc) FLR_FMA(da) FLR_FMA(t1) FLR_FMA(t2)
+                                 FLR_FMA(t3) FLR_FMA(t4)
+                         : [acc] "+v"(acc), [da] "+v"(da), [db] "+v"(db), [dc] "+v"(dc)
+                         : [x2] "v"(xv[2]), [x3] "v"(xv[3]), [j2] "v"(v[p][2]), [j3] "v"(v[p][3]), [L0] "n"(p),
+                           [w] "n"(cnt), [t0] "v"(FLR_T(0)), [t1] "v"(FLR_T(1)), [t2] "v"(FLR_T(2)),
+                           [t3] "v"(FLR_T(3)), [t4] "v"(FLR_T(4)));
+        }
+#undef FLR_T8
+#undef FLR_T
+        static_for(
+            [&readq](auto E) {
+              constexpr int q = done + decltype(E)::value;
+              if constexpr (4 * q + 3 < n0 + G * ND && q + RQ < NQT) readq(std::integral_constant<int, q + RQ>{});
+            },
+            std::make_integer_sequence<int, (G * ND + 3) / 4 + 1>{});
+      },
+      std::make_integer_sequence<int, Pt::PPC / G>{});
+  return acc;
+}
+#undef FLR_SUB
+#undef FLR_FMA
+
+template <bool DIAG, int NST = NSTAGE, bool TWO = false, int DM = 0>
 __device__ __forceinline__ void ref_chain_tile(float* lds, const Tile T, const int c, const float* __restrict__ Xc,
-                                               int64_t ldc, int K, int64_t steps, int first,
-                                               float* __restrict__ A) {
+                                               int64_t ldc, int K, int64_t steps, int first, float* __restrict__ A,
+                                               const float* __restrict__ Tc = nullptr, int nneg = 0) {
   using S = Staging<DIAG>;
   static_assert(!(TWO && DIAG), "two chains per lane on off-diagonal tiles only");
   static_assert(NST % 2 == 0 && NST >= 4, "two register buffers");
+  constexpr int NT = [] {
+    if constexpr (DM != 0)
+      return DeadPat<DM>::NT;
+    else
+      return 0;
+  }();
+  constexpr int TCH = [] {
+    if constexpr (DM != 0)
+      return DeadPat<DM>::TCH;
+    else
+      return 0;
+  }();
+  static_assert(NT <= 2 && !(TWO && DM), "the dead stream's DMA statements below");
+  constexpr int STG = STAGE + NT * 256;
+  constexpr int ZERO = NST * STG;
+  static_assert((ZERO + NT * 256) * 4 <= NSTAGE * STAGE * 4, "inside the kernel's one LDS array");
+  static_assert((NST - 1) * STG * 4 < 65536, "ds_read_b128's 16-bit offset reaches every stage");
   constexpr int NXI = TWO ? 2 : 1;
-  constexpr int OPB = S::DPW + NXI;
+  constexpr int OPB = S::DPW + NT + NXI;
   static_assert((NST - 2) * OPB + NXI < 64, "vmcnt counts to 63");
   const int lane = threadIdx.x & 63, r = lane >> 4, jl = lane & 15;
   int i, j, srow;
@@ -404,6 +575,7 @@
     gj = gj < K ? gj : K - 1;
     voj[u] = (uint32_t)((int64_t)(gj - jrow0) * rs * 4 + 16 * ((lane % NQ) ^ slot_swz(s)) - 1024 * (u - 2) + 2048);
   }
+  const uint32_t vot = 16 * lane;
   const int irow0 = min(DIAG ? SB * T.X + IW * T.g : i - r, K - 1);
   const char* sbi = reinterpret_cast<const char*>(Xc + (int64_t)irow0 * rs + (int64_t)c * ldc);
   const uint32_t voi = (uint32_t)((int64_t)((i < K ? i : K - 1) - irow0) * rs * 4 + 16 * jl);
@@ -414,7 +586,7 @@
     const int64_t co = (int64_t)ch * CS * 4;
     if (FLR_REF_ABL == 3) return;
     const char* sb = sbj + co;
-    const uint32_t m = (uint32_t)(uintptr_t)lds + 4 * slot * STAGE + 2048;
+    const uint32_t m = (uint32_t)(uintptr_t)lds + 4 * slot * STG + 2048;
 #define FLR_DMA(n, off) "global_load_lds_dwordx4 %[v" #n "], %[sb] offset:" #off "\n\t"
     if constexpr (S::DPW == 5)
       asm volatile("s_mov_b32 m0, %[m]\n\ts_nop 0\n\t" FLR_DMA(0, -2048) FLR_DMA(1, -1024) FLR_DMA(2, 0)
@@ -431,6 +603,21 @@
                    : "memory");
 #undef FLR_DMA
     static_assert(S::DPW == 4 || S::DPW == 5, "the DMA statements above");
+    if constexpr (NT > 0) {
+      const char* st = reinterpret_cast<const char*>(Tc) + (int64_t)ch * TCH * 4;
+      const uint32_t mt = (uint32_t)(uintptr_t)lds + 4 * (slot * STG + STAGE);
+      if constexpr (NT == 2)
+        asm volatile("s_mov_b32 m0, %[m]\n\ts_nop 0\n\tglobal_load_lds_dwordx4 %[v], %[sb] offset:0\n\t"
+                     "global_load_lds_dwordx4 %[v], %[sb] offset:1024"
+                     :
+                     : [m] "s"(mt), [sb] "s"(st), [v] "v"(vot)
+                     : "memory");
+      else
+        asm volatile("s_mov_b32 m0, %[m]\n\ts_nop 0\n\tglobal_load_lds_dwordx4 %[v], %[sb] offset:0"
+                     :
+                     : [m] "s"(mt), [sb] "s"(st), [v] "v"(vot)
+                     : "memory");
+    }
     asm volatile("global_load_dwordx4 %0, %1, %2" : "=v"(x) : "v"(voi), "s"(sbi + co) : "memory");
     if constexpr (TWO) asm volatile("global_load_dwordx4 %0, %1, %2" : "=v"(x2) : "v"(voi2), "s"(sbi + co) : "memory");
   };
@@ -442,10 +629,22 @@
 #pragma unroll
     for (int q = 0; q < NQ; ++q)
       if (FLR_REF_ABL != 2)
-        asm volatile("ds_read_b128 %0, %1 offset:%2" : "=v"(v[q]) : "v"(a[q]), "n"(decltype(st)::value * STAGE * 4)
+        asm volatile("ds_read_b128 %0, %1 offset:%2" : "=v"(v[q]) : "v"(a[q]), "n"(decltype(st)::value * STG * 4)
                      : "memory");
   };
 
+  uint32_t ta[NST];
+  if constexpr (DM != 0) {
+    const bool mixed = valid && ((i < nneg) != (j < nneg));
+    static_assert(NT * 256 % 64 == 0, "the zero block in whole 16-B pieces per lane");
+#pragma unroll
+    for (int q = 0; q < NT * 256 / 256; ++q)
+      *reinterpret_cast<f32x4*>(lds + ZERO + 256 * q + 4 * lane) = f32x4{0.f, 0.f, 0.f, 0.f};
+    asm volatile("s_waitcnt lgkmcnt(0)" ::: "memory");
+#pragma unroll
+    for (int u = 0; u < NST; ++u)
+      ta[u] = (uint32_t)(uintptr_t)(mixed ? lds + u * STG + STAGE : lds + ZERO);
+  }
   f32x4 va[NQ], vb[NQ];
   f32x4 xs[NST], xs2[NST];
   auto body = [&](auto U, int ch, f32x4(&vc)[NQ], f32x4(&vn)[NQ]) {
@@ -458,7 +657,9 @@
     if constexpr (TWO) asm volatile("" : "+v"(xs2[u]));
     issue(ch + NST - 1, (u + NST - 1) % NST, xs[(u + NST - 1) % NST], xs2[(u + NST - 1) % NST]);
     rows(std::integral_constant<int, (u + 1) % NST>{}, vn, ra);
-    if constexpr (TWO)
+    if constexpr (DM != 0)
+      acc = dead_chunk<DM>(xs[u], vc, acc, ta[u]);
+    else if constexpr (TWO)
       chain_chunk2(xs[u], xs2[u], vc, acc, acc2);
     else if (FLR_REF_ABL != 5)
       acc = chain_chunk(xs[u], vc, acc);
@@ -491,6 +692,40 @@
     ref_chain_tile<true>(lds, T, c, Xc, ldc, K, steps, first, A);
   else
     ref_chain_tile<false>(lds, T, c, Xc, ldc, K, steps, first, A);
+}
+
+template <int DM>
+__global__ __launch_bounds__(64) void ref_chain_dead_kernel(const float* __restrict__ Xl, int64_t ldc,
+                                                            const float* __restrict__ Tb, int64_t ldt, int K,
+                                                            int nneg, int64_t steps, int first,
+                                                            float* __restrict__ A) {
+  __shared__ __attribute__((aligned(16))) float lds[NSTAGE * STAGE];
+  const int c = (int)(blockIdx.x & 7);
+  const Tile T = tile_of((int)(blockIdx.x >> 3));
+  const int lane = threadIdx.x & 63, r = lane >> 4, jl = lane & 15;
+  int i, j;
+  bool keep = true;
+  if (T.diag) {
+    const int a = IW * T.g + r, o = jl + 1;
+    i = SB * T.X + a;
+    j = SB * T.X + ((a + o) & (SB - 1));
+    keep = o < SB / 2 || a < SB / 2;
+  } else {
+    i = SB * T.X + IW * T.g + r;
+    j = SB * T.Y + JW * T.h + jl;
+  }
+  const bool mixed = keep && i < K && j < K && ((i < nneg) != (j < nneg));
+  const float* Tc = Tb + (int64_t)c * ldt;
+  if (__builtin_amdgcn_ballot_w64(mixed) == 0) {
+    if (T.diag)
+      ref_chain_tile<true>(lds, T, c, Xl, ldc, K, steps, first, A);
+    else
+      ref_chain_tile<false>(lds, T, c, Xl, ldc, K, steps, first, A);
+  } else if (T.diag) {
+    ref_chain_tile<true, NSTD, false, DM>(lds, T, c, Xl, ldc, K, steps, first, A, Tc, nneg);
+  } else {
+    ref_chain_tile<false, NSTD, false, DM>(lds, T, c, Xl, ldc, K, steps, first, A, Tc, nneg);
+  }
 }
 
 constexpr int NST2 = 4;
@@ -913,7 +1148,7 @@
 };
 __global__ void ref_finish_kernel(const float* __restrict__ A, int chains, const float* __restrict__ X,
                                   const TailCols tc, int K, int64_t P, int64_t ldx, int64_t R, int t0, int t1,
-                                  double* __restrict__ D) {
+                                  double* __restrict__ D, const int* __restrict__ dflag, int nneg) {
   const int64_t idx = (int64_t)blockIdx.x * blockDim.x + threadIdx.x;
   if (idx >= (int64_t)K * K) return;
   const int i = (int)(idx / K), j = (int)(idx % K);
@@ -946,6 +1181,7 @@
       s = __builtin_fmaf(d, d, s);
     }
     v = (double)sqrt_rn(s);
+    if (dflag && *dflag && ((i < nneg) == (j < nneg))) v = __builtin_nan("");
   }
   D[(int64_t)i * K + j] = v;
   D[(int64_t)j * K + i] = v;
@@ -968,7 +1204,8 @@
   const int64_t per_step = (K > QJ ? quad_rows(K) : K) * 8 * 4;
   const int64_t nseg = (per_step * Rc + XC_CAP - 1) / XC_CAP;
   const int64_t Rs = ((R + nseg - 1) / nseg + XC_GROUP - 1) / XC_GROUP * XC_GROUP;
-  return n + (size_t)(per_step * Rs + XC_SLACK + (K > QJ ? quad_slack(K) : 0));
+  const int64_t regions = K <= 512 ? 4 * P + (int64_t(4) << 20) + 40 * XC_GROUP * per_step : 0;
+  return n + (size_t)(per_step * Rs + XC_SLACK + (K > QJ ? quad_slack(K) : 0) + regions);
 }
 
 extern "C" int flr_pairwise_l2_reference_tiles(int64_t K) {
@@ -1008,9 +1245,50 @@
   return wr;
 }
 
+constexpr int DM_ONE = 0x1EF, DM_FOUR = 0x04F;
+struct DeadBlock {
+  bool fast = false;
+  DeadPlan live{}, deadp{};
+  int dm = 0;
+  int64_t r0 = 0, S = 0;
+  int64_t Ll = 0, Lp = 0;
+  int64_t ldt = 0, toff = 0;
+};
+static DeadBlock dead_block(int64_t off, int64_t co, int64_t ci, int64_t kk, uint64_t dm) {
+  DeadBlock b;
+  const int m = (int)(dm & 0x1ff);
+  if (kk != 9 || (m != DM_ONE && m != DM_FOUR) || off % 8 != 0 || (co * ci * 9) % 8 != 0) return b;
+  b.fast = true;
+  b.dm = m;
+  b.live.on = b.deadp.on = 1;
+  for (int w = 0; w < 9; ++w) {
+    const int t = 8 - w;
+    DeadPlan& p = ((m >> t) & 1) ? b.deadp : b.live;
+    const int n = ((m >> t) & 1) ? b.deadp.nd++ : b.live.nl++;
+    p.tap |= (uint64_t)t << (4 * n);
+    p.rank |= (uint64_t)n << (4 * t);
+  }
+  b.live.nd = b.deadp.nd;
+  b.deadp.nl = b.live.nl;
+  b.r0 = off / 8;
+  b.S = co * ci * 9 / 8;
+  const int64_t np = (b.S + 16) / 9;
+  b.Ll = np * b.live.nl;
+  b.Lp = (b.Ll + XC_GROUP - 1) / XC_GROUP * XC_GROUP;
+  const int64_t tch = CS / b.live.nl * b.deadp.nd, trip = (int64_t)NSTD * CS;
+  b.ldt = ((b.Ll + trip - 1) / trip * NSTD + NSTD) * tch + 512;
+  b.ldt = (b.ldt + 63) / 64 * 64;
+  return b;
+}
+struct Region {
+  int64_t a, b;
+  int blk;
+  int64_t pos;
+};
+
 static int run_chains(const float* X, int64_t K, int64_t steps_total, int64_t ldx, const int64_t* taps, int64_t ntaps,
                       const uint64_t* dead, const float* gdead, int64_t nneg, int first, float* A, void* ws,
-                      size_t ws_bytes, int t0, int t1, hipStream_t st) {
+                      size_t ws_bytes, int t0, int t1, hipStream_t st, const int** dflag) {
   const size_t na = a_bytes(K);
   if (ws_bytes < na) return FLR_ERR_WORKSPACE;
   const int64_t R = steps_total;
@@ -1055,48 +1333,134 @@
     return FLR_OK;
   }
   const int64_t per_step = K * 8 * 4;
-  const int64_t ldc = (int64_t)((ws_bytes - na - XC_SLACK) / (size_t)per_step) / XC_GROUP * XC_GROUP;
+  const bool all_tiles = t0 == 0 && t1 == ntiles_of((int)K);
+  const int nn = (int)std::min<int64_t>(nneg, K);
+  std::vector<DeadBlock> db((size_t)ntaps);
+  size_t tfloats = 0;
+  const char* skip_knob = flr::knob("FLR_REF_DEAD_SKIP");
+  if (dead && gdead && all_tiles && !use_two_chains(K) && !(skip_knob && skip_knob[0] == '0'))
+    for (int64_t b = 0; b < ntaps; ++b) {
+      db[(size_t)b] = dead_block(taps[4 * b], taps[4 * b + 1], taps[4 * b + 2], taps[4 * b + 3], dead[b]);
+      if (!db[(size_t)b].fast) continue;
+      db[(size_t)b].toff = (int64_t)tfloats;
+      tfloats += (size_t)(8 * db[(size_t)b].ldt);
+    }
+  size_t xc_end = ws_bytes;
+  if (tfloats > 0) {
+    const size_t tb = tfloats * 4 + 256;
+    if (ws_bytes >= na + (size_t)XC_SLACK + (size_t)(per_step * XC_GROUP) + tb + 256)
+      xc_end = (ws_bytes - tb) / 256 * 256;
+    else
+      for (auto& b : db) b.fast = false;
+  }
+  float* Tall = reinterpret_cast<float*>(reinterpret_cast<char*>(ws) + xc_end);
+  int* flag = reinterpret_cast<int*>(Tall + tfloats);
+  const int64_t ldc = (int64_t)((xc_end - na - XC_SLACK) / (size_t)per_step) / XC_GROUP * XC_GROUP;
   if (ldc < XC_GROUP) return FLR_ERR_WORKSPACE;
-  const int64_t nseg = (R + ldc - 1) / ldc;
-  const int64_t Rs = ((R + nseg - 1) / nseg + XC_GROUP - 1) / XC_GROUP * XC_GROUP;
-  float* Xc = reinterpret_cast<float*>(reinterpret_cast<char*>(ws) + na);
+  auto plan = [&](int64_t r0, int64_t steps, bool regions, std::vector<Region>& out) {
+    out.clear();
+    int64_t cur = r0, pos = 0;
+    auto live = [&](int64_t a, int64_t b) {
+      out.push_back({a, b, -1, pos});
+      pos += (b - a + XC_GROUP - 1) / XC_GROUP * XC_GROUP;
+    };
+    for (int64_t b = 0; regions && b < ntaps; ++b) {
+      const DeadBlock& d = db[(size_t)b];
+      if (!d.fast || d.r0 < cur || d.r0 + d.S > r0 + steps) continue;
+      if (d.r0 > cur) live(cur, d.r0);
+      out.push_back({d.r0, d.r0 + d.S, (int)b, pos});
+      pos += d.Lp;
+      cur = d.r0 + d.S;
+    }
+    if (cur < r0 + steps) live(cur, r0 + steps);
+    return pos;
+  };
+  std::vector<Region> regs;
+  int64_t nseg = (R + ldc - 1) / ldc;
+  if (tfloats > 0 && plan(0, R, true, regs) <= ldc) nseg = 1;
+  const int64_t Rs = nseg == 1 ? R : ((R + nseg - 1) / nseg + XC_GROUP - 1) / XC_GROUP * XC_GROUP;
+  float* Xc0 = reinterpret_cast<float*>(reinterpret_cast<char*>(ws) + na);
+  bool streams_made = false, started = false;
   for (int64_t seg = 0; seg < nseg; ++seg) {
-    const int64_t r0 = seg * Rs, steps = (R - r0 < Rs) ? R - r0 : Rs;
-    if (steps <= 0) break;
-    const WaveRuns runs = wave_runs(taps, ntaps, r0, steps);
-    int rc = FLR_OK;
-    if (runs.pre[runs.n] > 0) {
-      hipLaunchKernelGGL(chain_transpose_kernel, dim3((unsigned)((runs.pre[runs.n] + 3) / 4), (unsigned)K), dim3(256),
-                         0, st, X, ldx, r0, steps, ldc, Xc, runs);
-      if ((rc = launch_status("chain_transpose_kernel")) != FLR_OK) return rc;
-    }
-    for (int64_t b = 0; b < ntaps; ++b) {
-      const int64_t off = taps[4 * b], co = taps[4 * b + 1], ci = taps[4 * b + 2], kk = taps[4 * b + 3];
-      if (off + co * ci * kk <= 8 * r0 || off >= 8 * (r0 + steps)) continue;
-      const int64_t tiles = (co + TAP_CO - 1) / TAP_CO * ((ci + TAP_ROWS / kk - 1) / (TAP_ROWS / kk));
-      const bool vec = off % 4 == 0 && co % TAP_CO == 0;
-      auto kern = kk == 9 ? (vec ? tap_chain_kernel<9, true> : tap_chain_kernel<9, false>)
-                : kk == 1 ? (vec ? tap_chain_kernel<1, true> : tap_chain_kernel<1, false>)
-                          : (vec ? tap_chain_kernel<0, true> : tap_chain_kernel<0, false>);
-      const uint64_t dm = dead ? dead[b] : 0;
-      hipLaunchKernelGGL(kern, dim3((unsigned)tiles, (unsigned)K), dim3(256), 0, st, X, ldx, off, (int)co, (int)ci,
-                         (int)kk, r0, steps, ldc, Xc, dm ? gdead : nullptr, dm, (int)std::min<int64_t>(nneg, K));
-      if ((rc = launch_status("tap_chain_kernel")) != FLR_OK) return rc;
-    }
-    const int64_t padded = (steps + XC_GROUP - 1) / XC_GROUP * XC_GROUP;
-    if (padded > steps &&
-        hipMemset2DAsync(Xc + steps, (size_t)ldc * 4, 0, (size_t)(padded - steps) * 4, (size_t)(K * 8), st) != hipSuccess)
-      return FLR_ERR_HIP;
-    if (t0 == 0 && t1 == ntiles_of((int)K) && use_two_chains(K)) {
-      hipLaunchKernelGGL(ref_chain2_kernel, dim3(8 * ntiles2_of((int)K)), dim3(64), 0, st, Xc, ldc, (int)K, steps,
-                         (first && seg == 0) ? 1 : 0, A);
-      rc = launch_status("ref_chain2_kernel");
-    } else {
-      hipLaunchKernelGGL(ref_chain_kernel, dim3(8 * (t1 - t0)), dim3(64), 0, st, Xc, ldc, (int)K, steps, t0,
-                         (first && seg == 0) ? 1 : 0, A);
-      rc = launch_status("ref_chain_kernel");
-    }
-    if (rc != FLR_OK) return rc;
+    const int64_t sr0 = seg * Rs, ssteps = (R - sr0 < Rs) ? R - sr0 : Rs;
+    if (ssteps <= 0) break;
+    if (plan(sr0, ssteps, tfloats > 0, regs) > ldc) plan(sr0, ssteps, false, regs);
+    for (const Region& rg : regs) {
+      const int fst = (first && !started) ? 1 : 0;
+      started = true;
+      float* Xc = Xc0 + rg.pos;
+      int rc = FLR_OK;
+      if (rg.blk >= 0) {
+        const DeadBlock& d = db[(size_t)rg.blk];
+        const int64_t off = taps[4 * rg.blk], co = taps[4 * rg.blk + 1], ci = taps[4 * rg.blk + 2];
+        if (!streams_made) {
+          streams_made = true;
+          if (hipMemsetAsync(Tall, 0, tfloats * 4 + 4, st) != hipSuccess) return FLR_ERR_HIP;
+          for (int64_t b = 0; b < ntaps; ++b) {
+            const DeadBlock& e = db[(size_t)b];
+            if (!e.fast) continue;
+            const int64_t n = taps[4 * b + 1] * taps[4 * b + 2] * e.deadp.nd;
+            hipLaunchKernelGGL(dead_stream_kernel, dim3((unsigned)((n + 255) / 256)), dim3(256), 0, st, gdead,
+                               taps[4 * b], (int)taps[4 * b + 1], (int)taps[4 * b + 2], e.deadp, e.ldt, Tall + e.toff,
+                               flag);
+            if ((rc = launch_status("dead_stream_kernel")) != FLR_OK) return rc;
+          }
+          if (dflag) *dflag = flag;
+        }
+        const int64_t zs = d.S / 9 * d.live.nl;
+        hipLaunchKernelGGL(zero_slots_kernel, dim3((unsigned)(K * 8)), dim3(256), 0, st, Xc, ldc, d.live.nl, zs, d.Lp);
+        if ((rc = launch_status("zero_slots_kernel")) != FLR_OK) return rc;
+        const int64_t cit = TAP_ROWS / d.live.nl;
+        const int64_t tiles = (co + TAP_CO - 1) / TAP_CO * ((ci + cit - 1) / cit);
+        const bool vec = off % 4 == 0 && co % TAP_CO == 0;
+        auto kern = vec ? tap_chain_kernel<9, true, true> : tap_chain_kernel<9, false, true>;
+        hipLaunchKernelGGL(kern, dim3((unsigned)tiles, (unsigned)K), dim3(256), 0, st, X, ldx, off, (int)co, (int)ci, 9,
+                           d.r0, d.S, ldc, Xc, (const float*)nullptr, (uint64_t)d.dm, nn, d.live);
+        if ((rc = launch_status("tap_chain_kernel")) != FLR_OK) return rc;
+        if (d.dm == DM_ONE)
+          hipLaunchKernelGGL(ref_chain_dead_kernel<DM_ONE>, dim3(8 * (t1 - t0)), dim3(64), 0, st, Xc, ldc,
+                             Tall + d.toff, d.ldt, (int)K, nn, d.Ll, fst, A);
+        else
+          hipLaunchKernelGGL(ref_chain_dead_kernel<DM_FOUR>, dim3(8 * (t1 - t0)), dim3(64), 0, st, Xc, ldc,
+                             Tall + d.toff, d.ldt, (int)K, nn, d.Ll, fst, A);
+        if ((rc = launch_status("ref_chain_dead_kernel")) != FLR_OK) return rc;
+        continue;
+      }
+      const int64_t r0 = rg.a, steps = rg.b - rg.a;
+      const WaveRuns runs = wave_runs(taps, ntaps, r0, steps);
+      if (runs.pre[runs.n] > 0) {
+        hipLaunchKernelGGL(chain_transpose_kernel, dim3((unsigned)((runs.pre[runs.n] + 3) / 4), (unsigned)K), dim3(256),
+                           0, st, X, ldx, r0, steps, ldc, Xc, runs);
+        if ((rc = launch_status("chain_transpose_kernel")) != FLR_OK) return rc;
+      }
+      for (int64_t b = 0; b < ntaps; ++b) {
+        const int64_t off = taps[4 * b], co = taps[4 * b + 1], ci = taps[4 * b + 2], kk = taps[4 * b + 3];
+        if (off + co * ci * kk <= 8 * r0 || off >= 8 * (r0 + steps)) continue;
+        const int64_t tiles = (co + TAP_CO - 1) / TAP_CO * ((ci + TAP_ROWS / kk - 1) / (TAP_ROWS / kk));
+        const bool vec = off % 4 == 0 && co % TAP_CO == 0;
+        auto kern = kk == 9 ? (vec ? tap_chain_kernel<9, true> : tap_chain_kernel<9, false>)
+                  : kk == 1 ? (vec ? tap_chain_kernel<1, true> : tap_chain_kernel<1, false>)
+                            : (vec ? tap_chain_kernel<0, true> : tap_chain_kernel<0, false>);
+        const uint64_t dm = dead ? dead[b] : 0;
+        hipLaunchKernelGGL(kern, dim3((unsigned)tiles, (unsigned)K), dim3(256), 0, st, X, ldx, off, (int)co, (int)ci,
+                           (int)kk, r0, steps, ldc, Xc, dm ? gdead : nullptr, dm, nn, DeadPlan{});
+        if ((rc = launch_status("tap_chain_kernel")) != FLR_OK) return rc;
+      }
+      const int64_t padded = (steps + XC_GROUP - 1) / XC_GROUP * XC_GROUP;
+      if (padded > steps) {
+        hipLaunchKernelGGL(zero_slots_kernel, dim3((unsigned)(K * 8)), dim3(256), 0, st, Xc, ldc, 0, steps, padded);
+        if ((rc = launch_status("zero_slots_kernel")) != FLR_OK) return rc;
+      }
+      if (all_tiles && use_two_chains(K)) {
+        hipLaunchKernelGGL(ref_chain2_kernel, dim3(8 * ntiles2_of((int)K)), dim3(64), 0, st, Xc, ldc, (int)K, steps,
+                           fst, A);
+        rc = launch_status("ref_chain2_kernel");
+      } else {
+        hipLaunchKernelGGL(ref_chain_kernel, dim3(8 * (t1 - t0)), dim3(64), 0, st, Xc, ldc, (int)K, steps, t0, fst, A);
+        rc = launch_status("ref_chain_kernel");
+      }
+      if (rc != FLR_OK) return rc;
+    }
   }
   return FLR_OK;
 }
@@ -1135,9 +1499,10 @@
   const int ntiles = K > 1 ? ntiles_of((int)K) : 0;
   const int t0 = (int)(part * ntiles / nparts), t1 = (int)((part + 1) * ntiles / nparts);
   float* A = reinterpret_cast<float*>(ws);
+  const int* dflag = nullptr;
   if (K > 1 && R > 0 && t1 > t0 &&
       (rc = run_chains(X, K, R, ldx, taps, ntaps, any_dead ? dead : nullptr, gdead, nneg, 1, A, ws, ws_bytes, t0, t1,
-                       st)) != FLR_OK)
+                       st, &dflag)) != FLR_OK)
     return rc;
   TailCols tc;
   for (int64_t u = 8 * R; u < 8 * R + 8; ++u) {
@@ -1159,7 +1524,7 @@
     }
   const int64_t kk = K * K;
   hipLaunchKernelGGL(ref_finish_kernel, dim3((unsigned)((kk + 255) / 256)), dim3(256), 0, st, A, R > 0 ? 1 : 0, X, tc,
-                     (int)K, P, ldx, R, t0, t1, D);
+                     (int)K, P, ldx, R, t0, t1, D, dflag, (int)std::min<int64_t>(nneg, K));
   return launch_status("ref_finish_kernel");
 }
 
@@ -1200,7 +1565,7 @@
     return FLR_OK;
   }
   return run_chains(X, K, steps, ldx, taps, ntaps, nullptr, nullptr, 0, first, A, ws, ws_bytes, 0, ntiles_of((int)K),
-                    st);
+                    st, nullptr);
 }
 
 extern "C" int flr_pairwise_l2_reference_partial(const float* X, int64_t K, int64_t steps, int64_t ldx, int first,
@@ -1219,6 +1584,6 @@
   const int64_t kk = K * K;
   hipLaunchKernelGGL(ref_finish_kernel, dim3((unsigned)((kk + 255) / 256)), dim3(256), 0, as_stream(stream),
                      reinterpret_cast<const float*>(ws), chains ? 1 : 0, Xtail, tc, (int)K, ntail, ldx, (int64_t)0, 0,
-                     K > 1 ? ntiles_of((int)K) : 0, D);
+                     K > 1 ? ntiles_of((int)K) : 0, D, nullptr, 0);
   return launch_status("ref_finish_kernel");
 }
```

New measurement: 16.24 rounds/s, median of 6. +3.8%, better.
